# wangjiarui153/AIGV-Assessor

Measured on AMD Instinct MI355X. Metric: scored clips/sec (8-frame 448x448, InternVL2-8B stage-2 score eval), higher is better.
Workload: dtype bf16

## Files before the change

### aigv-assessor_amd/context.py

```python
from __future__ import annotations

import ctypes as C
from typing import Dict, Optional

import torch
import torch.nn.functional as F

from . import native
from .graphs import _PARKED_GRAPHS


def rope_tables(head_dim: int, theta: float, n_pos: int, max_pos: int = 32768, scaling: Optional[dict] = None,
                seq_len: Optional[int] = None):
    base = float(theta)
    if scaling is not None and scaling.get("type") == "dynamic" and seq_len is not None and seq_len > max_pos:
        f = float(scaling["factor"])
        base = base * ((f * seq_len / max_pos) - (f - 1)) ** (head_dim / (head_dim - 2))
    inv_freq = 1.0 / (base ** (torch.arange(0, head_dim, 2).float() / head_dim))
    t = torch.arange(n_pos).to(inv_freq.dtype)
    if scaling is not None and scaling.get("type") == "linear":
        t = t / float(scaling["factor"])
    freqs = torch.outer(t, inv_freq)
    return freqs.cos().to(torch.bfloat16).contiguous(), freqs.sin().to(torch.bfloat16).contiguous()

# ... 131 lines not shown
            if name.startswith("mlpscore.ln1"):
                continue
            if name == "vision_model.embeddings.position_embedding":
                put(name, resized_pos_table(p.data, v.image_size // v.patch_size, cfg.image_size // v.patch_size))
            else:
                put(name, p.data)
        if self.stage == 1:
            put("mlpscore.fc1.weight", torch.zeros(1, l.hidden_size, dtype=torch.bfloat16))
            put("mlpscore.fc1.bias", torch.zeros(1, dtype=torch.bfloat16))
        self._upload_rope()
        native.check(lib.aigv_finalize_weights(ctx), ctx)
        native.check(lib.aigv_set_precision(ctx, 1 if getattr(self, "_precision", "bf16") == "fp8" else 0), ctx)
        native.check(lib.aigv_set_gemm_mode(ctx, int(getattr(self, "_gemm_mode", -1))), ctx)
        native.check(lib.aigv_set_row_trimming(ctx, int(getattr(self, "_row_trim", True))), ctx)
        native.check(lib.aigv_set_attention_numerics(ctx, int(getattr(self, "_attn_numerics", 0))), ctx)
        self._dirty = False

    def __del__(self):
        try:
            _PARKED_GRAPHS.extend(v for v in getattr(self, "_graphs", {}).values() if isinstance(v, tuple))
        except Exception:
            pass
        try:
            if getattr(self, "_ctx", None) is not None:
                native.release("aigv_ctx_destroy", self._ctx)
        except Exception:
            pass

    def _ctx_set(self, entry: str, *args):
        lib, ctx = self._native()
        native.check(getattr(lib, entry)(ctx, *args), ctx)

    def set_precision(self, mode: str = "bf16"):
        self._drop_graphs()
        if mode not in ("bf16", "fp8"):
            raise ValueError("precision must be 'bf16' or 'fp8'")
        self._precision = mode
        if self._ctx is not None and not self._dirty:
            native.check(native.load().aigv_set_precision(self._ctx, 1 if mode == "fp8" else 0), self._ctx)

    def set_attention_numerics(self, mode: str = "fp32"):
        self._drop_graphs()
        if mode not in ("reference", "fp32"):
            raise ValueError("attention numerics must be 'reference' or 'fp32'")
        self._attn_numerics = 1 if mode == "reference" else 0
        self._ctx_set("aigv_set_attention_numerics", self._attn_numerics)

    def set_gemm_mode(self, mode: int = -1):
        self._drop_graphs()
        self._gemm_mode = int(mode)
        self._ctx_set("aigv_set_gemm_mode", int(mode))

    TUNE_KNOBS = {"gemm_mode": 0, "gemm256_order": 1, "gemm256_variant": 2, "attn_waves": 3, "skinny_p": 4, "body_tile": 5, "co_kmax": 6,
                  "tail_slices": 7, "attn_lead_key": 8, "decode_fused": 9, "decode_fp8": 10, "skinny_p8": 11, "fuse_tails": 12, "lone_body": 13}

    def tune(self, knob: str, value: int = -1):
        self._drop_graphs()
        self._ctx_set("aigv_ctx_tune", self.TUNE_KNOBS[knob], int(value))

    def set_row_trimming(self, on: bool = True):
        self._drop_graphs()
        self._row_trim = bool(on)
        self._ctx_set("aigv_set_row_trimming", int(on))
        self.drop_dead_tail = bool(on)

    def prof_enable(self, on: bool = True):
        self._drop_graphs()
        self._prof_on = bool(on)
        self._ctx_set("aigv_prof_enable", int(on))

    def prof_read(self) -> Dict[str, Dict[str, float]]:
        lib, ctx = self._native()
        out = {}
        for cls, name in enumerate(("gemm_llm", "attn_vit", "attn_llm", "skinny", "gemm_fp8", "gemm_vit")):
            n, ms, fl, by = C.c_int64(), C.c_double(), C.c_double(), C.c_double()
            native.check(lib.aigv_prof_read(ctx, cls, C.byref(n), C.byref(ms), C.byref(fl), C.byref(by)), ctx)
            out[name] = dict(launches=n.value, ms=ms.value, flops=fl.value, bytes=by.value)
        out["gemm"] = {k: out["gemm_llm"][k] + out["gemm_vit"][k] for k in out["gemm_llm"]}
        return out
```

### aigv-assessor_amd/csrc/ctx.h

```cpp
#pragma once
#include <hip/hip_runtime.h>

#include <algorithm>
#include <string>
#include <unordered_map>
#include <vector>

#include "../../include/aigv_amd.h"
#include "kernels.h"

namespace aigv {

struct DevBuf {
  void* p = nullptr;
  size_t bytes = 0;
};

struct VitLayer {
  const bf16_t *ls1, *ls2, *qkv_w, *qkv_b, *qn, *kn, *proj_w, *proj_b, *fc1_w, *fc1_b, *fc2_w, *fc2_b, *n1w, *n1b, *n2w, *n2b;
};
struct LlmLayer {
  const bf16_t *wqkv, *wo, *w13, *w2, *an, *fn;
};

struct LlmLayerFp8 {
  uint8_t *wqkv = nullptr, *wo = nullptr, *w13 = nullptr, *w2 = nullptr;
  float *s_wqkv = nullptr, *s_wo = nullptr, *s_w13 = nullptr, *s_w2 = nullptr;
};

struct ProfRec {
  int cls;
  hipEvent_t a, b;
  double flops, bytes;
};

struct RowPlan {
  struct Tiny { int row0, stride_rows, count; };
  std::vector<Tiny> tiny;
  int rows = 0, body_halves = 0, tail_halves = 0, tail_rows = 0;
  int32_t* d_tab = nullptr;
  int cap_halves = 0;
};

}

struct aigv_ctx {
  aigv_config cfg{};
  int device = 0;
  std::string err;
  std::unordered_map<std::string, aigv::DevBuf> w;
  std::vector<void*> allocs;
  std::vector<void*> ws_allocs;
  bool ws_phase = false;
  bool finalized = false;
  int np = 0, S = 0, Kp = 0, grid = 0, ntok = 0, proj_in = 0, qkv_out = 0, head_dim = 0, vit_head_dim = 0, g = 0;
  std::vector<aigv::VitLayer> vit;
  std::vector<aigv::LlmLayer> llm;
  const bf16_t *patch_w = nullptr, *patch_b = nullptr, *pos = nullptr, *cls_pos = nullptr;
  const bf16_t *tok_emb = nullptr, *final_norm = nullptr, *lm_head = nullptr, *rope_cos = nullptr, *rope_sin = nullptr;
  const bf16_t *p_ln_w[2] = {nullptr, nullptr}, *p_ln_b[2] = {nullptr, nullptr}, *p_w1[2] = {nullptr, nullptr},
               *p_b1[2] = {nullptr, nullptr}, *p_w2[2] = {nullptr, nullptr}, *p_b2[2] = {nullptr, nullptr};
  ScoreHeadArgs score{};
  bf16_t *v_col = nullptr, *v_x = nullptr, *v_t = nullptr, *v_qkv = nullptr, *v_ao = nullptr, *v_h = nullptr;
  int32_t* v_cu = nullptr;
  bf16_t *p_t = nullptr, *p_mid = nullptr;
  bf16_t *l_h = nullptr, *l_t = nullptr, *l_qkv = nullptr, *l_ao = nullptr, *l_ffn = nullptr, *l_rows = nullptr;
  int32_t *l_pos = nullptr, *l_seq = nullptr, *l_cu = nullptr, *l_rowidx = nullptr, *l_rowidx2 = nullptr, *l_kvlen = nullptr;
  unsigned long long* l_packed = nullptr;
  int32_t* l_neg1 = nullptr;
  bool fp8_llm = false;
  bool llm_lin_dirty = false;
  std::vector<aigv::LlmLayerFp8> llm8;
  uint8_t* q8 = nullptr;
  float* q8_scale = nullptr;
  aigv::RowPlan rp_vit, rp_llm;
  const aigv::RowPlan* cur_rp = nullptr;
  bool trim_last_layer = true;
  int attn_round_scores = AIGV_ATTENTION_NUMERICS_DEFAULT;
  int tune[AIGV_TUNE_COUNT];
  aigv_ctx() { std::fill(tune, tune + AIGV_TUNE_COUNT, -1); }
  size_t splitk_floats = 0;
  float* splitk_ws = nullptr;
  float* splitk_ws_vit = nullptr;
  bool on_vit_front = false;
  bf16_t* l_trim = nullptr;
  bf16_t* l_trim_h = nullptr;
  bf16_t* l_score_ws = nullptr;
  bf16_t* l_lp = nullptr;
  int lp_ldo = 0;
  bf16_t *kc = nullptr, *vc = nullptr;
  bf16_t *kc_alt = nullptr, *vc_alt = nullptr;
  int32_t* beam_ints = nullptr;
  uint64_t *kv_drop = nullptr, *kv_drop_alt = nullptr;
  int kv_drop_ld = 0;
  bool kv_masked = false;
  float* dec_ws = nullptr;
  float2* dec_lse = nullptr;
  bf16_t* dec_cand = nullptr;
  int32_t *dec_pos = nullptr, *dec_seq = nullptr, *dec_kvlen = nullptr, *dec_slot = nullptr;
  std::vector<int32_t> h_dec;
  std::vector<int32_t> h_pos, h_seq, h_rowidx, h_kvlen;
  int kv_seqs = 0;
  bool kv_valid = false;
  struct {
    bool armed = false;
    int n_rows = 0, n_seg = 0, ld_cached = 0;
    int32_t rows[AIGV_MAX_PROBE_ROWS];
    const int32_t *seg_new = nullptr, *seg_cached = nullptr;
    float* out = nullptr;
    float* tok = nullptr;
    int ld_tok = 0;
  } probe;
  struct {
    bool armed = false;
    const uint64_t* words = nullptr;
    const uint64_t* rows = nullptr;
    int ld = 0;
    int layer_begin = 0, layer_end = 0;
  } drop;
  struct {
    bool armed = false;
    int n_score = 0, n_token = 0;
    int32_t rows[2 * AIGV_MAX_LENS_ROWS];
    bf16_t *hidden = nullptr, *normed = nullptr;
    float* score = nullptr;
  } lens;
  int32_t* l_lensidx = nullptr;
  struct StreamRows {
// ... 72 lines not shown
    if (!on) return;
    hipEventRecord(r.b, s);
    c->recs.push_back(r);
  }
};

struct RowPlanScope {
  aigv_ctx* c;
  RowPlanScope(aigv_ctx* c_, const RowPlan* rp) : c(c_) { c->cur_rp = rp; }
  ~RowPlanScope() { c->cur_rp = nullptr; }
};

struct SplitkVitScope {
  aigv_ctx* c;
  explicit SplitkVitScope(aigv_ctx* c_) : c(c_) { c->on_vit_front = true; }
  ~SplitkVitScope() { c->on_vit_front = false; }
};

struct GemmClassScope {
  aigv_ctx* c;
  int keep;
  GemmClassScope(aigv_ctx* c_, int cls) : c(c_), keep(c_->gemm_cls) { c->gemm_cls = cls; }
  ~GemmClassScope() { c->gemm_cls = keep; }
};

struct Tune {
  int v[AIGV_TUNE_COUNT];
  constexpr int operator[](int knob) const { return v[knob]; }
};
extern Tune g_tune;
inline int tune_knob(const aigv_ctx* c, int knob) { return (c && c->tune[knob] >= 0) ? c->tune[knob] : g_tune.v[knob]; }
inline int resolved_gemm_mode(const aigv_ctx* c) { return tune_knob(c, AIGV_TUNE_GEMM_MODE); }
inline Tune tune_of(const aigv_ctx* c) {
  Tune t;
  for (int k = 0; k < AIGV_TUNE_COUNT; ++k) t.v[k] = tune_knob(c, k);
  return t;
}

GemmArgs gemm_args(const bf16_t* A, int lda, const bf16_t* W, int ldw, bf16_t* C, int ldc, int M, int N, int K);
int build_row_plan(aigv_ctx* c, RowPlan& rp, const int32_t* cu, int n_seq, hipStream_t s);
int launch_one(aigv_ctx* c, const GemmArgs& a, int epi, bool use256, hipStream_t s);
int run_gemm(aigv_ctx* c, const GemmArgs& a, int epi, hipStream_t s);
int run_gemm_rows(aigv_ctx* c, const GemmArgs& a, int epi, const RowPlan& rp, hipStream_t s);
int run_gemm_full(aigv_ctx* c, const GemmArgs& a, int epi, hipStream_t s);
int run_llm_gemm(aigv_ctx* c, const GemmArgs& a, int epi, hipStream_t s);
int run_gemm_fp8(aigv_ctx* c, const bf16_t* A, int lda, int K, const uint8_t* W8, const float* w_scale, bf16_t* C, int ldc, int T, int N,
                 int epi, const bf16_t* resid, int ldr, hipStream_t s);
const char* skinny_check(const bf16_t* x, int ldx, int R, const bf16_t* W, int ldw, int N, int K, const bf16_t* resid, int ldr,
                         const bf16_t* out, int ldo, int epi);
int run_skinny(aigv_ctx* c, const bf16_t* x, int ldx, int R, const bf16_t* W, int ldw, int N, int K, const bf16_t* bias,
               const bf16_t* resid, int ldr, bf16_t* out, int ldo, int epi, hipStream_t s, int p = 1);
constexpr size_t SPLITK_MAX_FLOATS = (size_t)64 << 20;
int splitk_scratch(aigv_ctx* c, size_t need_floats, float** out);

struct DisarmScope {
  aigv_ctx* c;
  explicit DisarmScope(aigv_ctx* c_) : c(c_) {}
  ~DisarmScope() { c->probe.armed = false; c->drop.armed = false; c->lens.armed = false; c->stream_cap.armed = false; c->stream_patch.armed = false;
                   c->head_cap.armed = false; c->head_patch.armed = false; c->head_scale.armed = false; }
};
int probe_plan(aigv_ctx* c, const char* op, const int32_t* cu, int B, const int32_t* off_host, ProbeArgs* out);
int probe_layer(aigv_ctx* c, const ProbeArgs& plan, int li, bool cache, hipStream_t s);
int stream_rows_check(aigv_ctx* c, const char* op, const int32_t* rows, int n, int T, int lo, int hi, int L);
extern double g_rate256;

}
```

### aigv-assessor_amd/csrc/dispatch.hip

```cpp
#include <atomic>
#include <mutex>

#include "ctx.h"

namespace aigv {

static GemmArgs tuned(const aigv_ctx* c, const GemmArgs& a) {
  GemmArgs b = a;
  b.order_sel = tune_knob(c, AIGV_TUNE_GEMM256_ORDER); b.variant_sel = tune_knob(c, AIGV_TUNE_GEMM256_VARIANT);
  return b;
}
double g_rate256 = 1.46;
constexpr double KT128 = 0.95, FIX128 = 6.0, LONE128 = 0.70, FIX256 = 9.0, LAUNCH_GAP = 2.0;

static std::atomic<unsigned> g_route{0};
static inline void took(unsigned bit) { g_route.fetch_or(bit, std::memory_order_relaxed); }

static double kt256() { return 2.0 * KT128 / g_rate256; }

static double t256(long row_tiles, int N, int nk) {
  if (row_tiles <= 0) return 0;
  const long tiles = row_tiles * (N / 256);
  return (double)((tiles + 255) / 256) * (nk * kt256() + FIX256);
}
static double t128_blocks(long blocks, double nk_each) {
  const double rt = nk_each * KT128 + FIX128;
  const long full = blocks / 512, part = blocks % 512;
  return full * rt + (part == 0 ? 0.0 : part <= 256 ? LONE128 * rt : rt);
}
static double t128(int rows, int N, int nk) { return rows <= 0 ? 0 : t128_blocks((long)((rows + 127) / 128) * (N / 128), nk); }
static double t_finalize(long rows, int N, int S) { return (double)rows * N * (4.0 * S + 4.0) / 3.0e6 + 3.0; }

constexpr int MAX_DEVICES = 64;
static float* g_op_splitk_ws[MAX_DEVICES] = {};
static std::mutex g_op_splitk_lock;

int splitk_scratch(aigv_ctx* c, size_t need_floats, float** out) {
  if (need_floats > SPLITK_MAX_FLOATS) return fail(c, AIGV_ERR_ARG, "split-K scratch: %zu floats exceed the planner's cap", need_floats);
  if (c) {
    if (need_floats > c->splitk_floats) return fail(c, AIGV_ERR_STATE, "split-K scratch: %zu floats exceed the context's %zu", need_floats, c->splitk_floats);
    *out = c->on_vit_front ? c->splitk_ws_vit : c->splitk_ws;
    return 0;
  }
  int dev = 0;
  HIPCHK(c, hipGetDevice(&dev));
  if (dev < 0 || dev >= MAX_DEVICES) return fail(c, AIGV_ERR_ARG, "device %d out of range", dev);
  std::lock_guard<std::mutex> g(g_op_splitk_lock);
  if (!g_op_splitk_ws[dev]) HIPCHK(c, hipMalloc((void**)&g_op_splitk_ws[dev], SPLITK_MAX_FLOATS * sizeof(float)));
  *out = g_op_splitk_ws[dev];
  return 0;
}
constexpr int SPLITS[] = {2, 3, 4, 6, 8};

static double best_split128(int rows, int N, int nk, int epi, int* S_out) {
  *S_out = 1;
  double best = t128(rows, N, nk);
  if (epi == EPI_PATCH) return best;
  const long tiles = (long)((rows + 127) / 128) * (N / 128);
  for (int S : SPLITS) {
    if (nk % S || nk / S < 4 || (size_t)S * rows * N > SPLITK_MAX_FLOATS) continue;
    const double t = t128_blocks(tiles * S, (double)nk / S) + t_finalize(rows, N, S) + LAUNCH_GAP;
    if (t < best) { best = t; *S_out = S; }
  }
  return best;
}
static double best_split256(long row_tiles, int N, int nk, int* S_out) {
  *S_out = 0;
  double best = 1e30;
  for (int S : SPLITS) {
    if (nk % S || nk / S < 4 || (size_t)S * row_tiles * 256 * N > SPLITK_MAX_FLOATS) continue;
    const long blocks = row_tiles * (N / 256) * S;
    const double t = (double)((blocks + 255) / 256) * ((double)nk / S * kt256() + FIX256) + t_finalize(row_tiles * 256, N, S) + LAUNCH_GAP;
    if (t < best) { best = t; *S_out = S; }
  }
  return best;
}

static int skinny_epi(int epi) {
  switch (epi) {
    case EPI_STORE: return SK_STORE;
    case EPI_GELU: return SK_GELU;
    case EPI_LS_RESID: return SK_LS_RESID;
    case EPI_RESID: return SK_RESID;
    case EPI_SWIGLU: return SK_SWIGLU;
  }
  return -1;
}
static double t_skinny(int rows, int N, int K) {
  if (rows <= 0) return 0;
  if (rows > 64 || K % 128) return 1e30;
// ... 137 lines not shown
      took(AIGV_ROUTE_SKINNY);
      hipError_t e = aigv_launch_skinny_gemm(bot.A, bot.lda, bot.M, bot.W, bot.ldw, bot.N, bot.K, bot.bias, bot.resid, bot.ldr,
                                            bot.C, bot.ldc, sk, s, bot.ls);
      if (e != hipSuccess) return fail(c, AIGV_ERR_HIP, "skinny remainder (M=%d N=%d K=%d): %s", bot.M, bot.N, bot.K, hipGetErrorString(e));
      return 0;
    }
    if (pl.last_slices > 1) return launch_splitk(c, bot, epi, pl.last_slices, false, s);
    return launch_one(c, bot, epi, false, s);
  }
  return 0;
}

constexpr int TINY_TAIL = 4;

int build_row_plan(aigv_ctx* c, RowPlan& rp, const int32_t* cu, int n_seq, hipStream_t s) {
  rp.tiny.clear();
  std::vector<int32_t> body, tail;
  bool uniform = true;
  for (int b = 1; b < n_seq; ++b) uniform = uniform && (cu[b + 1] - cu[b] == cu[1] - cu[0]);
  rp.tail_rows = 0;
  for (int b = 0; b < n_seq; ++b) {
    const int L = cu[b + 1] - cu[b], nb = L / 256, rem = L % 256, r0 = cu[b] + nb * 256;
    for (int j = 0; j < 2 * nb; ++j) { body.push_back(cu[b] + j * 128); body.push_back(128); }
    if (rem == 0) continue;
    if (rem <= TINY_TAIL) {
      if (!uniform) rp.tiny.push_back({r0, 1, rem});
      else if (b == 0)
        for (int j = 0; j < rem; ++j) rp.tiny.push_back({r0 + j, L, n_seq});
      continue;
    }
    tail.push_back(r0); tail.push_back(std::min(rem, 128));
    if (rem > 128) { tail.push_back(r0 + 128); tail.push_back(rem - 128); }
    rp.tail_rows += rem;
  }
  rp.body_halves = (int)body.size() / 2;
  rp.tail_halves = (int)tail.size() / 2;
  rp.rows = cu[n_seq];
  if (rp.body_halves + rp.tail_halves > rp.cap_halves)
    return fail(c, AIGV_ERR_STATE, "row plan: %d half tiles exceed the table's %d", rp.body_halves + rp.tail_halves, rp.cap_halves);
  body.insert(body.end(), tail.begin(), tail.end());
  if (!body.empty()) HIPCHK(c, aigv_launch_write_ints(body.data(), (int)body.size(), rp.d_tab, s));
  return 0;
}

static int tail_slices(int N, int K, int forced) {
  const int tn = N / 256, nk = K / 64;
  int best = 1;
  for (int S : {2, 4, 8})
    if (nk % S == 0 && nk / S >= 8 && 2 * tn * S <= 256) best = S;
  if (forced == 1 || (forced > 1 && nk % forced == 0 && nk / forced >= 4)) best = forced;
  return best;
}

static int launch_tab(aigv_ctx* c, const GemmArgs& a, int epi, const int32_t* tab, int halves, int rows, int S, hipStream_t s) {
  if (halves <= 0) return 0;
  GemmArgs b = tuned(c, a);
  b.row_tab = tab; b.tab_halves = halves;
  GEMM_PROF_ROWS(c, a, rows, s);
  if (S <= 1) {
    took(AIGV_ROUTE_TAB_256);
    HIPCHK(c, aigv_launch_gemm256(b, epi, s));
    return 0;
  }
  float* ws = nullptr;
  TRY(splitk_scratch(c, (size_t)S * ((halves + 1) / 2) * 256 * a.N, &ws));
  took(AIGV_ROUTE_TAB_SPLITK);
  HIPCHK(c, aigv_launch_gemm_splitk(b, epi, S, ws, s, true));
  return 0;
}

static int run_tiny_tails(aigv_ctx* c, const GemmArgs& a, int epi, const RowPlan& rp, hipStream_t s) {
  const int sk = skinny_epi(epi);
  for (const RowPlan::Tiny& t : rp.tiny) {
    if (sk < 0 || a.K % 128) return fail(c, AIGV_ERR_STATE, "no skinny form for epilogue %d / K=%d (tiny sequence tails)", epi, a.K);
    const size_t ldx = (size_t)t.stride_rows * a.lda, ldo = (size_t)t.stride_rows * a.ldc, ldr = (size_t)t.stride_rows * a.ldr;
    if (ldx > 0x7fffffffu || ldo > 0x7fffffffu || ldr > 0x7fffffffu) return fail(c, AIGV_ERR_STATE, "tiny-tail row stride overflows");
    for (int i0 = 0; i0 < t.count; i0 += 64) {
      const int R = std::min(64, t.count - i0);
      const size_t r0 = (size_t)t.row0 + (size_t)i0 * t.stride_rows;
      ProfScope ps(c, c ? c->gemm_cls : AIGV_PROF_GEMM, 2.0 * R * (double)a.N * a.K, 2.0 * (double)a.N * a.K, s);
      took(t.stride_rows == 1 ? AIGV_ROUTE_TINY : AIGV_ROUTE_TINY_STRIDED);
      hipError_t e = aigv_launch_skinny_gemm(a.A + r0 * a.lda, (int)ldx, R, a.W, a.ldw, a.N, a.K, a.bias, a.resid ? a.resid + r0 * a.ldr : nullptr,
                                            (int)ldr, a.C + r0 * a.ldc, (int)ldo, sk, s, a.ls, 0);
      if (e != hipSuccess) return fail(c, AIGV_ERR_HIP, "skinny tiny tails (R=%d N=%d K=%d): %s", R, a.N, a.K, hipGetErrorString(e));
    }
  }
  return 0;
}

int run_gemm_rows(aigv_ctx* c, const GemmArgs& a, int epi, const RowPlan& rp, hipStream_t s) {
  if (const char* m = aigv_gemm_check(a, epi)) return fail(c, AIGV_ERR_ARG, "%s (M=%d N=%d K=%d epi=%d)", m, a.M, a.N, a.K, epi);
  if (a.M != rp.rows) return fail(c, AIGV_ERR_STATE, "row plan covers %d rows, the GEMM has %d", rp.rows, a.M);
  const int mode = resolved_gemm_mode(c);
  if (mode == 3) return run_gemm(c, a, epi, s);
  if (mode == 4) return use_co(c, a, mode) ? launch_co(c, a, epi, s) : launch_one(c, a, epi, false, s);
  if (use_co(c, a, mode)) {
    if (rp.body_halves + rp.tail_halves > 0) {
      GemmArgs b = a;
      b.row_tab = rp.d_tab; b.tab_halves = rp.body_halves + rp.tail_halves;
      GEMM_PROF_ROWS(c, a, rp.body_halves * 128 + rp.tail_rows, s);
      took(AIGV_ROUTE_TAB_CO);
      HIPCHK(c, aigv_launch_gemmco(tuned(c, b), epi, s));
    }
    return run_tiny_tails(c, a, epi, rp, s);
  }
  if (mode == 1 || a.N < 256) return launch_one(c, a, epi, false, s);
  if (mode == 2 && a.N % 256 == 0) return launch_one(c, a, epi, true, s);
  if (a.N % 256) {
    if (epi == EPI_SWIGLU) return launch_one(c, a, epi, false, s);
    TRY(run_gemm_rows(c, col_slice(a, 0, a.N - 128), epi, rp, s));
    return launch_one(c, col_slice(a, a.N - 128, 128), epi, false, s);
  }
  const int S = tail_slices(a.N, a.K, tune_knob(c, AIGV_TUNE_TAIL_SLICES));
  const bool body128 = rp.body_halves > 0 && tune_knob(c, AIGV_TUNE_BODY_TILE) == 2;
  const bool tails_apart = rp.tail_halves > 0 && S > 1;
  const long body_tiles = (long)(rp.body_halves / 2) * (a.N / 256);
  const int lone_knob = tune_knob(c, AIGV_TUNE_LONE_BODY);
  const bool lone = !body128 && lone_knob != 1 && rp.body_halves > 0 && a.N % 128 == 0 &&
                    (lone_knob == 2 || (body_tiles <= 128 && (!tails_apart || a.K / 64 >= 128) && (lone_knob != 3 || tails_apart) && (lone_knob != 4 || !tails_apart)));
  if (lone) {
    GemmArgs b = tuned(c, a);
    b.row_tab = rp.d_tab; b.tab_halves = tails_apart ? rp.body_halves : rp.body_halves + rp.tail_halves;
    b.variant_sel = 7;
    GEMM_PROF_ROWS(c, a, rp.body_halves * 128 + (tails_apart ? 0 : rp.tail_rows), s);
    took(AIGV_ROUTE_TAB_LONE);
    HIPCHK(c, aigv_launch_gemmco(b, epi, s));
  } else if (body128) {
    {
      GemmArgs b = a;
      b.row_tab = rp.d_tab; b.tab_halves = rp.body_halves;
      GEMM_PROF_ROWS(c, a, rp.body_halves * 128, s);
      took(AIGV_ROUTE_TAB_128);
      HIPCHK(c, aigv_launch_gemm(b, epi, s));
    }
    if (rp.tail_halves > 0 && !tails_apart) TRY(launch_tab(c, a, epi, rp.d_tab + 2 * rp.body_halves, rp.tail_halves, rp.tail_rows, 1, s));
  } else if (!tails_apart) {
    TRY(launch_tab(c, a, epi, rp.d_tab, rp.body_halves + rp.tail_halves, rp.body_halves * 128 + rp.tail_rows, 1, s));
  } else {
    const int tn = a.N / 256;
    const long body_wg = (long)(rp.body_halves / 2) * tn, slice_wg = (long)((rp.tail_halves + 1) / 2) * tn * S;
    const size_t need = (size_t)S * ((rp.tail_halves + 1) / 2) * 256 * a.N;
    const int fuse_knob = tune_knob(c, AIGV_TUNE_FUSE_TAILS);
    const bool by_fill = body_wg % 256 != 0 && body_wg % 256 + slice_wg <= 320;
    if (!lone && rp.body_halves > 0 && (rp.body_halves & 1) == 0 && need <= (c ? c->splitk_floats : SPLITK_MAX_FLOATS) && fuse_knob != 1 && (by_fill || fuse_knob == 2)) {
      float* ws = nullptr;
      TRY(splitk_scratch(c, need, &ws));
      GemmArgs b = tuned(c, a);
      b.row_tab = rp.d_tab; b.tab_halves = rp.body_halves; b.fuse_tail_halves = rp.tail_halves; b.part = ws; b.k_slices = S;
      GEMM_PROF_ROWS(c, a, rp.body_halves * 128 + rp.tail_halves * 128, s);
      took(AIGV_ROUTE_TAB_FUSED);
      HIPCHK(c, aigv_launch_gemm256_fused(b, epi, s));
      GemmArgs f = a;
      f.row_tab = rp.d_tab + 2 * rp.body_halves; f.tab_halves = rp.tail_halves;
      HIPCHK(c, aigv_launch_gemm_finalize(f, epi, S, ws, s));
      return run_tiny_tails(c, a, epi, rp, s);
    }
    if (!lone) TRY(launch_tab(c, a, epi, rp.d_tab, rp.body_halves, rp.body_halves * 128, 1, s));
  }
  if (tails_apart) {
    const size_t per_pair = (size_t)S * 256 * a.N;
    const size_t cap = c ? c->splitk_floats : SPLITK_MAX_FLOATS;
    const int max_halves = (int)std::min<size_t>(cap / per_pair, 4096) * 2;
    if (max_halves < 2) return fail(c, AIGV_ERR_STATE, "split-K scratch too small for one tail tile (N=%d, %d slices)", a.N, S);
    for (int h0 = 0; h0 < rp.tail_halves; h0 += max_halves) {
      const int nh = std::min(max_halves, rp.tail_halves - h0);
      TRY(launch_tab(c, a, epi, rp.d_tab + 2 * (rp.body_halves + h0), nh, nh * 128, S, s));
    }
  }
  return run_tiny_tails(c, a, epi, rp, s);
}

int run_gemm_full(aigv_ctx* c, const GemmArgs& a, int epi, hipStream_t s) {
  if (const char* m = aigv_gemm_check(a, epi)) return fail(c, AIGV_ERR_ARG, "%s (M=%d N=%d K=%d epi=%d)", m, a.M, a.N, a.K, epi);
  const int mode = resolved_gemm_mode(c);
  if (use_co(c, a, mode)) return launch_co(c, a, epi, s);
  if (mode == 1 || a.N < 256 || (a.N % 256 && epi == EPI_SWIGLU)) return launch_one(c, a, epi, false, s);
  if (a.N % 256) {
    TRY(launch_one(c, col_slice(a, 0, a.N - 128), epi, true, s));
    return launch_one(c, col_slice(a, a.N - 128, 128), epi, false, s);
  }
  return launch_one(c, a, epi, true, s);
}

int run_llm_gemm(aigv_ctx* c, const GemmArgs& a, int epi, hipStream_t s) {
  return c->cur_rp ? run_gemm_rows(c, a, epi, *c->cur_rp, s) : run_gemm(c, a, epi, s);
}

GemmArgs gemm_args(const bf16_t* A, int lda, const bf16_t* W, int ldw, bf16_t* C, int ldc, int M, int N, int K) {
  GemmArgs a{};
  a.A = A; a.lda = lda; a.W = W; a.ldw = ldw; a.C = C; a.ldc = ldc; a.M = M; a.N = N; a.K = K;
  return a;
}

int run_gemm_fp8(aigv_ctx* c, const bf16_t* A, int lda, int K, const uint8_t* W8, const float* w_scale, bf16_t* C, int ldc, int T, int N,
                 int epi, const bf16_t* resid, int ldr, hipStream_t s) {
  hipError_t e = hipSuccess;
  if (A) {
    e = aigv_launch_quant_fp8_rows(A, lda, T, K, c->q8, K, c->q8_scale, s);
    if (e != hipSuccess) return fail(c, AIGV_ERR_HIP, "fp8 activation quantisation (T=%d K=%d): %s", T, K, hipGetErrorString(e));
  }
  GemmArgs a = tuned(c, GemmArgs{});
  a.A = (const bf16_t*)c->q8; a.lda = K; a.W = (const bf16_t*)W8; a.ldw = K; a.C = C; a.ldc = ldc; a.M = T; a.N = N; a.K = K;
  a.row_scale = c->q8_scale; a.col_scale = w_scale; a.resid = resid; a.ldr = ldr;
  ProfScope ps(c, AIGV_PROF_GEMM_FP8, 2.0 * T * (double)N * K, (double)T * K + (double)N * K + 2.0 * T * (epi == EPI_SWIGLU ? N / 2 : N), s);
  e = aigv_launch_gemm256_fp8(a, epi, s);
  if (e != hipSuccess) return fail(c, e == hipErrorInvalidValue ? AIGV_ERR_ARG : AIGV_ERR_HIP, "fp8 gemm (M=%d N=%d K=%d epi=%d): %s", T, N, K, epi, hipGetErrorString(e));
  return 0;
}


const char* skinny_check(const bf16_t* x, int ldx, int R, const bf16_t* W, int ldw, int N, int K, const bf16_t* resid, int ldr,
                         const bf16_t* out, int ldo, int epi) {
  if (R < 0 || N <= 0 || K <= 0) return "skinny gemm: empty problem";
  if (R > 64) return "skinny gemm: more than 64 rows";
  if (K % 128) return "skinny gemm: K must be a multiple of 128";
  if (!x || !W || !out) return "skinny gemm: null operand";
  if (ldx < K || ldw < K || (ldx % 8) || (ldw % 8)) return "skinny gemm: bad leading dimension (ldx and ldw: at least K, multiples of 8)";
  const int n_out = epi == SK_SWIGLU ? N / 2 : N;
  if (ldo < n_out) return "skinny gemm: ldo is below the output width (rows would overlap)";
  if (ldo % 4) return "skinny gemm: ldo must be a multiple of 4 (the kernel stores 8 bytes at out + row * ldo + n)";
  if ((epi == SK_RESID || epi == SK_LS_RESID) && !resid) return "skinny gemm: residual epilogue needs resid";
  if (resid && ldr < n_out) return "skinny gemm: ldr is below the width of the residual rows";
  if (resid && (ldr % 4)) return "skinny gemm: ldr must be a multiple of 4 (the kernel reads 8 bytes at resid + row * ldr + n)";
  return nullptr;
}

int run_skinny(aigv_ctx* c, const bf16_t* x, int ldx, int R, const bf16_t* W, int ldw, int N, int K, const bf16_t* bias,
               const bf16_t* resid, int ldr, bf16_t* out, int ldo, int epi, hipStream_t s, int p) {
  if (const char* m = skinny_check(x, ldx, R, W, ldw, N, K, resid, ldr, out, ldo, epi))
    return fail(c, AIGV_ERR_ARG, "%s (R=%d N=%d K=%d epi=%d)", m, R, N, K, epi);
  ProfScope ps(c, AIGV_PROF_SKINNY, 2.0 * R * (double)N * K, 2.0 * (double)N * K, s);
  hipError_t e = aigv_launch_skinny_gemm(x, ldx, R, W, ldw, N, K, bias, resid, ldr, out, ldo, epi, s, nullptr, p);
  if (e != hipSuccess) return fail(c, e == hipErrorInvalidValue ? AIGV_ERR_ARG : AIGV_ERR_HIP,
                                   "skinny gemm (R=%d N=%d K=%d epi=%d): %s", R, N, K, epi, hipGetErrorString(e));
  return 0;
}

}

using namespace aigv;

extern "C" int aigv_plan_gemm(int M, int N, int K, int epi, int* plan, double* est_us) {
  if (!plan || M <= 0 || N <= 0 || K <= 0 || N % 128 || K % 64 || epi < 0 || epi >= EPI_COUNT)
    return fail(nullptr, AIGV_ERR_ARG, "aigv_plan_gemm: bad problem M=%d N=%d K=%d epi=%d", M, N, K, epi);
  const int pmode = g_tune[AIGV_TUNE_GEMM_MODE] == 3 ? 0 : g_tune[AIGV_TUNE_GEMM_MODE];
  const int right = split_columns(M, N, K, epi, pmode);
  const GemmPlan pl = plan_gemm(M, N - right, K, epi, pmode);
  plan[6] = right;
  plan[0] = pl.top_tiles; plan[1] = pl.mid_tiles; plan[2] = pl.mid_slices; plan[3] = pl.last_rows; plan[4] = pl.last_kind;
  plan[5] = pl.last_slices;
  if (est_us) *est_us = pl.est_us + (right ? t128(M, right, K / 64) + LAUNCH_GAP : 0.0);
  return 0;
}

extern "C" int aigv_gemm_route(int clear) {
  return (int)(clear ? g_route.exchange(0, std::memory_order_relaxed) : g_route.load(std::memory_order_relaxed));
}
```

### aigv-assessor_amd/csrc/kernels.h

```cpp
#pragma once
#include <hip/hip_runtime.h>
#include <stdint.h>

typedef uint16_t bf16_t;

enum GemmEpilogue {
  EPI_STORE = 0,
  EPI_GELU = 1,
  EPI_LS_RESID = 2,
  EPI_RESID = 3,
  EPI_SWIGLU = 4,
  EPI_PATCH = 5,
  EPI_COUNT = 6,
  EPI_PARTIAL = 6
};

struct GemmArgs {
  const bf16_t* A; int lda;
  const bf16_t* W; int ldw;
  bf16_t* C; int ldc;
  const bf16_t* bias;
  const bf16_t* ls;
  const bf16_t* resid; int ldr;
  const bf16_t* pos;
  int M, N, K;
  int np;
  float* part;
  int k_slices;
  const float* row_scale;
  const float* col_scale;
  const int32_t* row_tab; int tab_halves;
  int fuse_tail_halves, fuse_body_wg;
  int order_sel, variant_sel;
  int order;
};

const char* aigv_gemm_check(const GemmArgs& a, int epi);
hipError_t aigv_launch_gemm(const GemmArgs& a, int epi, hipStream_t s);
hipError_t aigv_launch_gemm_splitk(const GemmArgs& a, int epi, int k_slices, float* ws, hipStream_t s, bool tile256 = false);
hipError_t aigv_launch_gemm256_partial(const GemmArgs& a, hipStream_t s);
hipError_t aigv_launch_gemm256_fp8(const GemmArgs& a, int epi, hipStream_t s);
hipError_t aigv_launch_gemm256_fp8_partial(const GemmArgs& a, hipStream_t s);
hipError_t aigv_launch_gemm_splitk_fp8(const GemmArgs& a, int epi, int k_slices, float* ws, hipStream_t s);
hipError_t aigv_launch_rmsnorm_quant_fp8(const bf16_t* x, int ldx, const bf16_t* w, uint8_t* q, int ldq, float* scale, int rows, int H, float eps,
                                         hipStream_t s);
hipError_t aigv_launch_quant_fp8_rows(const bf16_t* x, int ldx, int rows, int K, uint8_t* q, int ldq, float* scale, hipStream_t s);
bool aigv_gemm256_supported(const GemmArgs& a);
hipError_t aigv_launch_gemm256_fused(const GemmArgs& a, int epi, hipStream_t s);
hipError_t aigv_launch_gemm_finalize(const GemmArgs& a, int epi, int k_slices, const float* ws, hipStream_t s);
hipError_t aigv_launch_gemm256(const GemmArgs& a, int epi, hipStream_t s);
bool aigv_gemmco_supported(const GemmArgs& a);
hipError_t aigv_launch_gemmco(const GemmArgs& a, int epi, hipStream_t s);

struct AttnArgsUnmasked {
  const bf16_t* q; int ldq;
  const bf16_t* k; int ldk;
  const bf16_t* v; int ldv;
  bf16_t* o; int ldo;
  const int32_t* cu;
  int n_seq, max_len;
  int n_heads, n_kv_heads;
  int q_group_stride, kv_head_stride;
  int kv_len_offset;
  const int32_t* kv_off;
  size_t kv_seq_stride;
  int causal;
  float post_div;
  int round_scores;
  float q_prescale;
  const int32_t* rope_pos; const bf16_t* rope_cos; const bf16_t* rope_sin;
  int rope_pos_is_row;
  int q_tail;
  int uniform_len;
  int waves;
  int lead_key;
  int q_begin;
};
struct AttnArgsKeyDrop : AttnArgsUnmasked {
  const uint64_t* key_drop;
  int ld_drop;
};
struct AttnArgs : AttnArgsKeyDrop {
  const uint64_t* drop_rows;
};
const char* aigv_attn_check(const AttnArgs& a, int head_dim);
hipError_t aigv_launch_attention(const AttnArgs& a, int head_dim, hipStream_t s);
constexpr int AIGV_DECODE_KEYS_PER_CHUNK = 128;
constexpr int AIGV_DECODE_MAX_CHUNKS = 2048;
size_t aigv_attention_decode_ws_floats(int n_seq, int n_kv, int g, int cap);
hipError_t aigv_launch_attention_decode(const bf16_t* q, int ldq, int q_group_stride, const bf16_t* kc,
                                        const bf16_t* vc, const int32_t* kv_lens, int cap, bf16_t* o, int ldo,
                                        int n_seq, int n_kv, int g, int head_dim, float post_div, int max_kv_len,
                                        float* ws, hipStream_t s, const uint64_t* key_drop = nullptr, int ld_drop = 0);

#ifndef AIGV_MAX_ATTN_SEGMENTS
#define AIGV_MAX_ATTN_SEGMENTS 64
#endif
#ifndef AIGV_MAX_PROBE_ROWS
#define AIGV_MAX_PROBE_ROWS 64
#endif
#ifndef AIGV_MAX_KV_CAPACITY
#define AIGV_MAX_KV_CAPACITY 262144
#endif
struct ProbeRow { int32_t row, row0, seq, off; };
struct ProbeRowTab { ProbeRow r[AIGV_MAX_PROBE_ROWS]; };
struct ProbeArgs {
  const bf16_t* q; int ldq;
  const bf16_t* k; int ldk;
  int n_heads, n_kv_heads;
  int q_group_stride, kv_head_stride;
  size_t kv_seq_stride;
  float post_div;
  const bf16_t* rope_cos; const bf16_t* rope_sin;
  const int32_t* seg_new; const int32_t* seg_cached; int ld_cached;
  int n_seg;
  float* out; size_t out_row_stride;
  int n_rows;
  ProbeRowTab tab;
  float* tok; int ld_tok; size_t tok_row_stride;
};
const char* aigv_probe_check(const ProbeArgs& a, int head_dim, int total_rows, int max_pos);
hipError_t aigv_launch_attention_probe(const ProbeArgs& a, int head_dim, hipStream_t s);

hipError_t aigv_launch_layernorm(const bf16_t* x, int ldx, const bf16_t* w, const bf16_t* b, bf16_t* y, int ldy,
                                 int rows, int H, float eps, hipStream_t s);
hipError_t aigv_launch_rmsnorm(const bf16_t* x, int ldx, const bf16_t* w, bf16_t* y, int ldy, int rows, int H,
                               float eps, const int32_t* row_idx, hipStream_t s);
hipError_t aigv_launch_pixel_shuffle(const bf16_t* vit, int grid, int Hv, bf16_t* out, int frames, hipStream_t s);
hipError_t aigv_launch_im2col(const bf16_t* frames, int F, int C, int S, int P, int Kp, bf16_t* out, hipStream_t s);
hipError_t aigv_launch_gather_rows(const bf16_t* src, int ld, const int32_t* idx, int n, bf16_t* dst, int H, hipStream_t s);
hipError_t aigv_launch_lens_tap(const bf16_t* src, int ld, const int32_t* idx, int n, const bf16_t* w, bf16_t* raw, bf16_t* normed, int H, float eps,
                                hipStream_t s);
hipError_t aigv_launch_scatter_rows(const bf16_t* src, const int32_t* idx, int n, bf16_t* dst, int ld, int H, hipStream_t s);
hipError_t aigv_launch_stream_rows(bf16_t* stream, int ld, const int32_t* idx, int n, bf16_t* side, int n_depths, int depth, int H, bool to_stream,
                                   hipStream_t s);
#define AIGV_MAX_HEAD_BITS 64
enum { HEAD_CAPTURE = 0, HEAD_PATCH = 1, HEAD_SCALE = 2 };
struct HeadScales { float v[AIGV_MAX_HEAD_BITS]; };
hipError_t aigv_launch_head_rows(bf16_t* ao, int ld, const int32_t* idx, int n, bf16_t* side, int n_layers, int layer, int n_heads, int D, int mode,
                                 uint64_t heads, const float* scale, hipStream_t s);
hipError_t aigv_launch_cls_rows(const bf16_t* cls_pos, bf16_t* x, int F, int tokens_per_frame, int H, hipStream_t s);
hipError_t aigv_launch_rope(bf16_t* qkv, int ld, const int32_t* pos, const bf16_t* cos, const bf16_t* sin,
                            int tokens, int n_rot, int slots, int n_groups, int D, hipStream_t s, int first_rot = 0);
hipError_t aigv_launch_embed(const int64_t* ids, const int32_t* slot, const bf16_t* emb, const bf16_t* vis,
                             const bf16_t* motion, int n_vis, bf16_t* out, int tokens, int H, hipStream_t s);
enum { SK_STORE = 0, SK_RESID = 1, SK_SWIGLU = 2, SK_GELU = 3, SK_ARGMAX = 4, SK_RELU = 5, SK_LS_RESID = 6, SK_ROPE_KV = 7, SK_ARGMAX_LSE = 8, SK_ARGMAX_LSE_STORE = 9 };
hipError_t aigv_launch_skinny_gemm(const bf16_t* x, int ldx, int R, const bf16_t* W, int ldw, int N, int K,
                                   const bf16_t* bias, const bf16_t* resid, int ldr, bf16_t* out, int ldo, int epi,
                                   hipStream_t s, const bf16_t* ls = nullptr, int p = 1);
struct AigvRopeKv {
  const int32_t* pos; const int32_t* seq;
  const bf16_t* cos; const bf16_t* sin;
  bf16_t* kc; bf16_t* vc;
  int g, n_kv, cap;
};
bool aigv_skinny_fp8_supported(int K, bool with_norm);
hipError_t aigv_launch_skinny_fp8(const bf16_t* x, int ldx, int R, const uint8_t* W8, int ldw, const float* w_scale, int N, int K, const bf16_t* resid,
                                  int ldr, bf16_t* out, int ldo, int epi, const AigvRopeKv* rk, const bf16_t* norm_w, float eps, int p, hipStream_t s);
bool aigv_skinny_norm_fusable(int K);
hipError_t aigv_launch_skinny_swiglu_normed(const bf16_t* x, int ldx, int R, const bf16_t* W, int ldw, int N, int K, bf16_t* out, int ldo,
                                            const bf16_t* norm_w, float norm_eps, hipStream_t s, int p = 1);
hipError_t aigv_launch_skinny_rope_kv(const bf16_t* x, int ldx, int R, const bf16_t* W, int ldw, int N, int K, bf16_t* qkv, int ldo,
                                      const int32_t* pos, const int32_t* seq, const bf16_t* cos, const bf16_t* sin, bf16_t* kc, bf16_t* vc,
                                      int g, int n_kv, int cap, int head_dim, hipStream_t s, const bf16_t* norm_w = nullptr, float norm_eps = 0.f, int p = 1);
hipError_t aigv_launch_lm_head_argmax(const bf16_t* h, int R, int H, const bf16_t* W, int V,
                                      unsigned long long* packed, int64_t* out_idx, float* out_val, hipStream_t s);
#ifndef AIGV_MAX_CANDIDATES
#define AIGV_MAX_CANDIDATES 64
#endif
#ifndef AIGV_MAX_TOPK
#define AIGV_MAX_TOPK 16
#endif
size_t aigv_lm_head_lse_slots(int V);
size_t aigv_cand_logit_elems(int R);
hipError_t aigv_launch_lm_head_argmax_logprob(const bf16_t* h, int R, int H, const bf16_t* W, int V, unsigned long long* packed, float2* part,
                                              int64_t* out_idx, float* out_val, float* out_logprob, hipStream_t s, const int64_t* cand = nullptr,
                                              int C = 0, bf16_t* cand_logit = nullptr, float* out_cand = nullptr, int k = 0,
                                              bf16_t* row_logit = nullptr, int ldl = 0, int64_t* top_ids = nullptr, float* top_logprob = nullptr);
size_t aigv_topk_logit_ld(int V);
hipError_t aigv_launch_lm_head_lse_partials(const bf16_t* h, int R, int H, const bf16_t* W, int V, unsigned long long* packed, float2* part,
                                            hipStream_t s, bf16_t* logits = nullptr, int ldl = 0);
hipError_t aigv_launch_lm_head_logits(const bf16_t* h, int R, int H, const bf16_t* W, int V, bf16_t* out, int ldo, hipStream_t s,
                                      bool one_form = false, int ldh = 0);
hipError_t aigv_launch_label_logprob(const bf16_t* logits, int rows, int V, int ldo, const int64_t* labels, float* out, hipStream_t s);
hipError_t aigv_launch_cand_logprob(const bf16_t* logits, int rows, int V, int ldo, const int64_t* cand, int C, float* out, hipStream_t s);
hipError_t aigv_launch_topk_logprob(const bf16_t* logits, int rows, int V, int ldo, int k, int64_t* top_ids, float* top_logprob, hipStream_t s);
struct ScoreHeadArgs {
  const bf16_t* x; int ldx; int B;
  int n_layers; int dims[9];
  const bf16_t* w[8]; const bf16_t* b[8];
  float* score;
};
hipError_t aigv_launch_score_head(const ScoreHeadArgs& a, bf16_t* scratch, hipStream_t s);
hipError_t aigv_launch_score_head_groups(const ScoreHeadArgs& a, int G, size_t group_stride, bf16_t* scratch, hipStream_t s);
hipError_t aigv_launch_kv_store(const bf16_t* qkv, int ld, const int32_t* seq_of_tok, const int32_t* pos,
                                bf16_t* kc, bf16_t* vc, int tokens, int n_groups, int g, int D, int cap,
// ... 19 lines not shown
```

### aigv-assessor_amd/csrc/ops.hip

```cpp
#include "ctx.h"

using namespace aigv;

extern "C" {

int aigv_op_gemm(const void* A, int lda, const void* W_, int ldw, void* C, int ldc, const void* bias, const void* ls,
                 const void* resid, int ldr, const void* pos, int np, int M, int N, int K, int epi, void* stream) {
  GemmArgs a = gemm_args((const bf16_t*)A, lda, (const bf16_t*)W_, ldw, (bf16_t*)C, ldc, M, N, K);
  a.bias = (const bf16_t*)bias; a.ls = (const bf16_t*)ls; a.resid = (const bf16_t*)resid; a.ldr = ldr;
  a.pos = (const bf16_t*)pos; a.np = np;
  return run_gemm(nullptr, a, epi, (hipStream_t)stream);
}

int aigv_op_gemm_check(const void* A, int lda, const void* W_, int ldw, const void* C, int ldc, const void* bias, const void* ls,
                       const void* resid, int ldr, const void* pos, int np, int M, int N, int K, int epi) {
  GemmArgs a = gemm_args((const bf16_t*)A, lda, (const bf16_t*)W_, ldw, (bf16_t*)C, ldc, M, N, K);
  a.bias = (const bf16_t*)bias; a.ls = (const bf16_t*)ls; a.resid = (const bf16_t*)resid; a.ldr = ldr;
  a.pos = (const bf16_t*)pos; a.np = np;
  if (const char* m = aigv_gemm_check(a, epi)) return fail(nullptr, AIGV_ERR_ARG, "%s (M=%d N=%d K=%d epi=%d)", m, M, N, K, epi);
  return 0;
}

int aigv_op_skinny_gemm_check(const void* x, int ldx, int R, const void* W_, int ldw, int N, int K, const void* resid, int ldr,
                              const void* out, int ldo, int epi) {
  if (const char* m = skinny_check((const bf16_t*)x, ldx, R, (const bf16_t*)W_, ldw, N, K, (const bf16_t*)resid, ldr, (const bf16_t*)out, ldo, epi))
    return fail(nullptr, AIGV_ERR_ARG, "%s (R=%d N=%d K=%d epi=%d)", m, R, N, K, epi);
  return 0;
}

int aigv_op_gemm_rows(const void* A, int lda, const void* W_, int ldw, void* C, int ldc, const void* bias, const void* ls,
                      const void* resid, int ldr, const int32_t* cu_host, int n_seq, int N, int K, int epi, void* stream) {
  if (!cu_host || n_seq < 1 || cu_host[0] != 0) return fail(nullptr, AIGV_ERR_ARG, "aigv_op_gemm_rows: bad cu_seqlens");
  for (int b = 0; b < n_seq; ++b)
    if (cu_host[b + 1] <= cu_host[b]) return fail(nullptr, AIGV_ERR_ARG, "aigv_op_gemm_rows: empty sequence %d", b);
  if (epi == EPI_PATCH) return fail(nullptr, AIGV_ERR_ARG, "aigv_op_gemm_rows: no patch epilogue");
  const int M = cu_host[n_seq];
  GemmArgs a = gemm_args((const bf16_t*)A, lda, (const bf16_t*)W_, ldw, (bf16_t*)C, ldc, M, N, K);
  a.bias = (const bf16_t*)bias; a.ls = (const bf16_t*)ls; a.resid = (const bf16_t*)resid; a.ldr = ldr;
  RowPlan rp;
  rp.cap_halves = M / 128 + 2 * n_seq + 2;
  HIPCHK(nullptr, hipMalloc((void**)&rp.d_tab, (size_t)2 * rp.cap_halves * sizeof(int32_t)));
  int rc = build_row_plan(nullptr, rp, cu_host, n_seq, (hipStream_t)stream);
  if (!rc) rc = run_gemm_rows(nullptr, a, epi, rp, (hipStream_t)stream);
  hipStreamSynchronize((hipStream_t)stream);
  hipFree(rp.d_tab);
  return rc;
}

int aigv_op_gemm_splitk(const void* A, int lda, const void* W_, int ldw, void* C, int ldc, const void* bias, const void* ls,
                        const void* resid, int ldr, int M, int N, int K, int epi, int k_slices, void* ws_f32, void* stream) {
  GemmArgs a = gemm_args((const bf16_t*)A, lda, (const bf16_t*)W_, ldw, (bf16_t*)C, ldc, M, N, K);
  a.bias = (const bf16_t*)bias; a.ls = (const bf16_t*)ls; a.resid = (const bf16_t*)resid; a.ldr = ldr;
  if (const char* m = aigv_gemm_check(a, epi)) return fail(nullptr, AIGV_ERR_ARG, "%s", m);
  hipError_t e = aigv_launch_gemm_splitk(a, epi, k_slices, (float*)ws_f32, (hipStream_t)stream);
  if (e != hipSuccess) return fail(nullptr, e == hipErrorInvalidValue ? AIGV_ERR_ARG : AIGV_ERR_HIP, "split-K gemm: %s", hipGetErrorString(e));
  return 0;
}

int aigv_op_gemm_splitk256(const void* A, int lda, const void* W_, int ldw, void* C, int ldc, const void* bias, const void* ls,
                           const void* resid, int ldr, int M, int N, int K, int epi, int k_slices, void* ws_f32, void* stream) {
  GemmArgs a = gemm_args((const bf16_t*)A, lda, (const bf16_t*)W_, ldw, (bf16_t*)C, ldc, M, N, K);
  a.bias = (const bf16_t*)bias; a.ls = (const bf16_t*)ls; a.resid = (const bf16_t*)resid; a.ldr = ldr;
  if (const char* m = aigv_gemm_check(a, epi)) return fail(nullptr, AIGV_ERR_ARG, "%s", m);
  hipError_t e = aigv_launch_gemm_splitk(a, epi, k_slices, (float*)ws_f32, (hipStream_t)stream, true);
  if (e != hipSuccess) return fail(nullptr, e == hipErrorInvalidValue ? AIGV_ERR_ARG : AIGV_ERR_HIP, "split-K gemm (256 tile): %s", hipGetErrorString(e));
  return 0;
}

int aigv_op_quant_fp8_rows(const void* x_bf16, int ldx, int rows, int K, void* q_e4m3, int ldq, float* row_scale, void* stream) {
  hipError_t e = aigv_launch_quant_fp8_rows((const bf16_t*)x_bf16, ldx, rows, K, (uint8_t*)q_e4m3, ldq, row_scale, (hipStream_t)stream);
  if (e != hipSuccess) return fail(nullptr, e == hipErrorInvalidValue ? AIGV_ERR_ARG : AIGV_ERR_HIP, "fp8 row quantisation (rows=%d K=%d): %s", rows, K, hipGetErrorString(e));
  return 0;
}

int aigv_op_gemm_fp8(const void* A_e4m3, int lda, const void* W_e4m3, int ldw, void* C, int ldc, const float* row_scale,
                     const float* col_scale, const void* bias, const void* ls, const void* resid, int ldr, int M, int N, int K, int epi,
                     int k_slices, void* ws_f32, void* stream) {
  GemmArgs a{};
  a.A = (const bf16_t*)A_e4m3; a.lda = lda; a.W = (const bf16_t*)W_e4m3; a.ldw = ldw; a.C = (bf16_t*)C; a.ldc = ldc;
  a.M = M; a.N = N; a.K = K; a.bias = (const bf16_t*)bias; a.row_scale = row_scale; a.col_scale = col_scale;
  a.ls = (const bf16_t*)ls; a.resid = (const bf16_t*)resid; a.ldr = ldr;
  const int n_out = epi == EPI_SWIGLU ? N / 2 : N;
  if (ldc < n_out || (ldc % 8) || lda < K || ldw < K)
    return fail(nullptr, AIGV_ERR_ARG, "aigv_op_gemm_fp8: bad leading dimension (M=%d N=%d K=%d)", M, N, K);
  hipError_t e = k_slices > 1 ? aigv_launch_gemm_splitk_fp8(a, epi, k_slices, (float*)ws_f32, (hipStream_t)stream)
                              : aigv_launch_gemm256_fp8(a, epi, (hipStream_t)stream);
  if (e != hipSuccess)
    return fail(nullptr, e == hipErrorInvalidValue ? AIGV_ERR_ARG : AIGV_ERR_HIP,
                "fp8 gemm (M=%d N=%d K=%d epi=%d; needs N %% 256 == 0, K %% 128 == 0, 16-byte row strides, both scale vectors, epi in "
                "{store, gelu, ls_resid, resid, swiglu}): %s", M, N, K, epi, hipGetErrorString(e));
  return 0;
}

int aigv_op_skinny_gemm(const void* x, int ldx, int R, const void* W_, int ldw, int N, int K, const void* bias,
                        const void* resid, int ldr, void* out, int ldo, int epi, void* stream) {
  return run_skinny(nullptr, (const bf16_t*)x, ldx, R, (const bf16_t*)W_, ldw, N, K, (const bf16_t*)bias,
                    (const bf16_t*)resid, ldr, (bf16_t*)out, ldo, epi, (hipStream_t)stream, g_tune[AIGV_TUNE_SKINNY_P] ? g_tune[AIGV_TUNE_SKINNY_P] : 1);
}

// ... 600 lines not shown
```

### aigv-assessor_amd/csrc/passes.hip

```cpp
#include <cmath>

#include "ctx.h"

using namespace aigv;

namespace aigv {
int stream_rows_check(aigv_ctx* c, const char* op, const int32_t* rows, int n, int T, int lo, int hi, int L) {
  if (lo < 0 || lo > hi || hi > L) return fail(c, AIGV_ERR_ARG, "%s: depths [%d, %d) outside 0 <= lo <= hi <= %d", op, lo, hi, L);
  for (int i = 0; i < n; ++i) {
    if (rows[i] < 0 || rows[i] >= T) return fail(c, AIGV_ERR_ARG, "%s: row %d (packed row %d) outside [0, %d), the rows the pass runs", op, i, rows[i], T);
    if (i > 0 && rows[i] <= rows[i - 1])
      return fail(c, AIGV_ERR_ARG, "%s: rows %d and %d (packed rows %d, %d) are not strictly ascending", op, i - 1, i, rows[i - 1], rows[i]);
  }
  return 0;
}
}

extern "C" {

static int vit_norm(aigv_ctx* c, const bf16_t* x, const bf16_t* w, const bf16_t* b, bf16_t* y, int rows, hipStream_t s) {
  const aigv_config& k = c->cfg;
  if (k.vit_norm_rms) HIPCHK(c, aigv_launch_rmsnorm(x, k.vit_hidden, w, y, k.vit_hidden, rows, k.vit_hidden, k.vit_eps, nullptr, s));
  else HIPCHK(c, aigv_launch_layernorm(x, k.vit_hidden, w, b, y, k.vit_hidden, rows, k.vit_hidden, k.vit_eps, s));
  return 0;
// ... 116 lines not shown
  const aigv_config& k = c->cfg;
  const int H = k.llm_hidden, Md = k.motion_dim;
  if ((size_t)n_clips * Md > (size_t)k.vit_chunk * c->ntok * c->proj_in || n_clips > k.vit_chunk * c->ntok)
    return fail(c, AIGV_ERR_STATE, "motion batch does not fit the projector workspace");
  HIPCHK(c, aigv_launch_layernorm((const bf16_t*)motion_feature, Md, c->p_ln_w[1], c->p_ln_b[1], c->p_t, Md, n_clips, Md, 1e-5f, s));
  for (int r0 = 0; r0 < n_clips; r0 += 64) {
    const int R = std::min(64, n_clips - r0);
    TRY(run_skinny(c, c->p_t + (size_t)r0 * Md, Md, R, c->p_w1[1], Md, H, Md, c->p_b1[1], nullptr, 0,
                   c->p_mid + (size_t)r0 * H, H, SK_GELU, s, 0));
    TRY(run_skinny(c, c->p_mid + (size_t)r0 * H, H, R, c->p_w2[1], H, H, H, c->p_b2[1], nullptr, 0,
                   (bf16_t*)out + (size_t)r0 * H, H, SK_STORE, s, 0));
  }
  return 0;
}

static int upload_out_rows(aigv_ctx* c, const int32_t* score_rows, bool with_score, int B, const int32_t* logit_rows, int R,
                           int total_rows, hipStream_t s) {
  const aigv_config& k = c->cfg;
  if (R > k.max_out_rows) return fail(c, AIGV_ERR_ARG, "%d logit rows exceed max_out_rows %d", R, k.max_out_rows);
  c->h_rowidx.clear();
  for (int i = 0; i < (with_score ? B : 0); ++i) c->h_rowidx.push_back(score_rows[i]);
  for (int i = 0; i < R; ++i) c->h_rowidx.push_back(logit_rows[i]);
  for (int v : c->h_rowidx)
    if (v < 0 || v >= total_rows) return fail(c, AIGV_ERR_ARG, "output row index %d outside 0..%d", v, total_rows - 1);
  if (!c->h_rowidx.empty()) HIPCHK(c, aigv_launch_write_ints(c->h_rowidx.data(), (int)c->h_rowidx.size(), c->l_rowidx, s));
  return 0;
}

static int final_rows(aigv_ctx* c, float* score, int B, int R, int64_t* argmax, const bf16_t* hidden, bool compact, hipStream_t s) {
  const aigv_config& k = c->cfg;
  const int H = k.llm_hidden;
  const int nS = score ? B : 0;
  const int n = nS + R;
  if (n == 0) return 0;
  HIPCHK(c, aigv_launch_rmsnorm(hidden, H, c->final_norm, c->l_rows, H, n, H, k.rms_eps, compact ? nullptr : c->l_rowidx, s));
  for (int b0 = 0; b0 < nS; b0 += 64) {
    ScoreHeadArgs a = c->score;
    a.x = c->l_rows + (size_t)b0 * H; a.ldx = H; a.B = std::min(64, nS - b0); a.score = score + b0;
    HIPCHK(c, aigv_launch_score_head(a, c->l_score_ws, s));
  }
  for (int r0 = 0; r0 < R; r0 += 64) {
    const int rr = std::min(64, R - r0);
    ProfScope ps(c, AIGV_PROF_SKINNY, 2.0 * rr * (double)k.vocab * H, 2.0 * (double)k.vocab * H, s);
    HIPCHK(c, aigv_launch_lm_head_argmax(c->l_rows + (size_t)(nS + r0) * H, rr, H, c->lm_head, k.vocab, c->l_packed,
                                         argmax + r0, nullptr, s));
  }
  return 0;
}

static int llm_layer_qkv(aigv_ctx* c, int li, int T, hipStream_t s) {
  const aigv_config& k = c->cfg;
  const LlmLayer& L = c->llm[li];
  const int H = k.llm_hidden, D = c->head_dim, g = c->g, nkv = k.llm_kv_heads;
  if (c->fp8_llm) {
    HIPCHK(c, aigv_launch_rmsnorm_quant_fp8(c->l_h, H, L.an, c->q8, H, c->q8_scale, T, H, k.rms_eps, s));
    TRY(run_gemm_fp8(c, nullptr, H, H, c->llm8[li].wqkv, c->llm8[li].s_wqkv, c->l_qkv, c->qkv_out, T, c->qkv_out, EPI_STORE, nullptr, 0, s));
  } else {
    HIPCHK(c, aigv_launch_rmsnorm(c->l_h, H, L.an, c->l_t, H, T, H, k.rms_eps, nullptr, s));
    TRY(run_llm_gemm(c, gemm_args(c->l_t, H, L.wqkv, H, c->l_qkv, c->qkv_out, T, c->qkv_out, H), EPI_STORE, s));
  }
  HIPCHK(c, aigv_launch_rope(c->l_qkv, c->qkv_out, c->l_pos, c->rope_cos, c->rope_sin, T, 1, g + 2, nkv, D, s, g));
  return 0;
}

static int llm_layer_post(aigv_ctx* c, int li, int T, hipStream_t s) {
  const aigv_config& k = c->cfg;
  const LlmLayer& L = c->llm[li];
  const int H = k.llm_hidden, I = k.llm_inter;
  if (c->fp8_llm && li != k.llm_layers - 1) {
    const LlmLayerFp8& Q = c->llm8[li];
    TRY(run_gemm_fp8(c, c->l_ao, H, H, Q.wo, Q.s_wo, c->l_h, H, T, H, EPI_RESID, c->l_h, H, s));
    HIPCHK(c, aigv_launch_rmsnorm_quant_fp8(c->l_h, H, L.fn, c->q8, H, c->q8_scale, T, H, k.rms_eps, s));
    TRY(run_gemm_fp8(c, nullptr, H, H, Q.w13, Q.s_w13, c->l_ffn, I, T, 2 * I, EPI_SWIGLU, nullptr, 0, s));
    TRY(run_gemm_fp8(c, c->l_ffn, I, I, Q.w2, Q.s_w2, c->l_h, H, T, H, EPI_RESID, c->l_h, H, s));
    return 0;
  }
  {
    GemmArgs a = gemm_args(c->l_ao, H, L.wo, H, c->l_h, H, T, H, H);
    a.resid = c->l_h; a.ldr = H;
    TRY(run_llm_gemm(c, a, EPI_RESID, s));
  }
  HIPCHK(c, aigv_launch_rmsnorm(c->l_h, H, L.fn, c->l_t, H, T, H, k.rms_eps, nullptr, s));
  TRY(run_llm_gemm(c, gemm_args(c->l_t, H, L.w13, H, c->l_ffn, I, T, 2 * I, H), EPI_SWIGLU, s));
  GemmArgs a = gemm_args(c->l_ffn, I, L.w2, I, c->l_h, H, T, H, I);
  a.resid = c->l_h; a.ldr = H;
  TRY(run_llm_gemm(c, a, EPI_RESID, s));
  return 0;
}

static int upload_decode_state(aigv_ctx* c, int N, hipStream_t s) {
  c->h_dec.resize((size_t)4 * N);
  for (int i = 0; i < N; ++i) {
    const int len = c->h_kvlen[i];
    c->h_dec[i] = len; c->h_dec[N + i] = i; c->h_dec[2 * N + i] = len + 1; c->h_dec[3 * N + i] = -1;
  }
  HIPCHK(c, aigv_launch_write_ints(c->h_dec.data(), N, c->dec_pos, s));
  HIPCHK(c, aigv_launch_write_ints(c->h_dec.data() + N, N, c->dec_seq, s));
  HIPCHK(c, aigv_launch_write_ints(c->h_dec.data() + 2 * N, N, c->dec_kvlen, s));
  HIPCHK(c, aigv_launch_write_ints(c->h_dec.data() + 3 * N, N, c->dec_slot, s));
  c->kv_seqs = N;
  return 0;
}

static AttnArgs llm_attn_args(const aigv_ctx* c, int B) {
  const aigv_config& k = c->cfg;
  const int D = c->head_dim;
  AttnArgs a{};
  a.q = c->l_qkv; a.ldq = c->qkv_out;
  a.o = c->l_ao; a.ldo = k.llm_hidden;
  a.cu = c->l_cu; a.n_seq = B;
  a.n_heads = k.llm_heads; a.n_kv_heads = k.llm_kv_heads;
  a.q_group_stride = (c->g + 2) * D;
  a.causal = 1; a.post_div = sqrtf((float)D); a.q_prescale = 1.0f;
  a.round_scores = c->attn_round_scores; a.waves = tune_knob(c, AIGV_TUNE_ATTN_WAVES);
  a.rope_pos = c->l_pos; a.rope_cos = c->rope_cos; a.rope_sin = c->rope_sin;
  a.rope_pos_is_row = 1;
  return a;
}

int aigv_llm_prefill(aigv_ctx* c, const int64_t* ids, const int32_t* slot, const int32_t* cu, int B, const void* vis,
                     int n_vis, const void* motion, const int32_t* score_rows, float* score, const int32_t* logit_rows,
                     int R, int64_t* argmax, int keep_kv, void* stream) {
  if (!c || !ids || !slot || !cu) return fail(c, AIGV_ERR_ARG, "aigv_llm_prefill: null argument");
  const bool probing = c->probe.armed;
  const bool dropping = c->drop.armed;
  const bool lensing = c->lens.armed;
  const bool patching = c->stream_patch.armed;
  const bool capturing = c->stream_cap.armed;
  const bool h_scaling = c->head_scale.armed, h_patching = c->head_patch.armed, h_capturing = c->head_cap.armed;
  DisarmScope disarm(c);
  if (!c->finalized) return fail(c, AIGV_ERR_STATE, "aigv_llm_prefill: call aigv_finalize_weights first");
  if (dropping && probing) return fail(c, AIGV_ERR_ARG, "aigv_llm_prefill: a key-drop mask and the score-attention probe are both armed: the probe does not know the mask");
  const aigv_config& k = c->cfg;
  if (dropping && (c->drop.layer_begin < 0 || c->drop.layer_begin > c->drop.layer_end || c->drop.layer_end > k.llm_layers))
    return fail(c, AIGV_ERR_ARG, "aigv_llm_prefill: key-drop mask armed for layers [%d, %d), outside 0 <= begin <= end <= %d", c->drop.layer_begin, c->drop.layer_end, k.llm_layers);
  if (dropping && keep_kv && (c->drop.rows || c->drop.layer_begin != 0 || c->drop.layer_end != k.llm_layers))
    return fail(c, AIGV_ERR_ARG, "aigv_llm_prefill: keep_kv under a key-drop mask with row words or a partial layer window (aigv_key_drop_arm_ex): the mask kept "
                                 "beside the KV cache has neither");
  if (B <= 0 || B > k.max_seqs) return fail(c, AIGV_ERR_ARG, "n_clips %d outside 1..%d", B, k.max_seqs);
// ... 53 lines not shown
    }
  }
  HIPCHK(c, hipSetDevice(c->device));
  hipStream_t s = (hipStream_t)stream;
  const int H = k.llm_hidden, I = k.llm_inter, D = c->head_dim, g = c->g, nkv = k.llm_kv_heads;

  if (B + 1 > AIGV_SMALL_INTS / 2) return fail(c, AIGV_ERR_ARG, "at most %d clips per prefill call", AIGV_SMALL_INTS / 2 - 1);
  HIPCHK(c, aigv_launch_seqpos(cu, B, c->l_pos, c->l_seq, c->l_cu, T, s));
  TRY(build_row_plan(c, c->rp_llm, cu, B, s));
  RowPlanScope rps(c, &c->rp_llm);

  HIPCHK(c, aigv_launch_embed(ids, slot, c->tok_emb, (const bf16_t*)vis, (const bf16_t*)motion, n_vis, c->l_h, T, H, s));
  TRY(upload_out_rows(c, score_rows, score != nullptr, B, logit_rows, R, T, s));
  const int32_t* lens_idx = c->l_lensidx;
  auto lens_tap = [&](int depth, const bf16_t* src, const int32_t* idx) -> int {
    const size_t off = (size_t)depth * n_lens * H;
    HIPCHK(c, aigv_launch_lens_tap(src, H, idx, n_lens, c->final_norm, c->lens.hidden + off, c->lens.normed + off, H, k.rms_eps, s));
    return 0;
  };
  if (patching) HIPCHK(c, aigv_launch_write_ints(sp.rows.data(), (int)sp.rows.size(), c->l_streamidx, s));
  if (capturing) HIPCHK(c, aigv_launch_write_ints(sc.rows.data(), (int)sc.rows.size(), c->l_streamidx + k.max_tokens, s));
  if (h_scaling && !hs.all_rows) HIPCHK(c, aigv_launch_write_ints(hs.rows.data(), (int)hs.rows.size(), c->l_headidx, s));
  if (h_patching) HIPCHK(c, aigv_launch_write_ints(hp.rows.data(), (int)hp.rows.size(), c->l_headidx + k.max_tokens, s));
  if (h_capturing) HIPCHK(c, aigv_launch_write_ints(hc.rows.data(), (int)hc.rows.size(), c->l_headidx + 2 * (size_t)k.max_tokens, s));
  if (lensing) {
    HIPCHK(c, aigv_launch_write_ints(c->lens.rows, n_lens, c->l_lensidx, s));
    HIPCHK(c, aigv_launch_write_ints(lens_at, n_lens, c->l_lensidx + 2 * AIGV_MAX_LENS_ROWS, s));
  }
  const int n_out = (int)c->h_rowidx.size();
  int q_tail = 0;
  constexpr int TRIM_ROWS = 16;
  std::vector<int32_t> small_rows;
  {
    std::vector<int> per_clip(B, 0), clip_of(c->h_rowidx.size());
    for (size_t i = 0; i < c->h_rowidx.size(); ++i) {
      int b = 0;
      while (cu[b + 1] <= c->h_rowidx[i]) ++b;
      clip_of[i] = b;
      ++per_clip[b];
      q_tail = std::max(q_tail, cu[b + 1] - c->h_rowidx[i]);
    }
    for (size_t i = 0; i < c->h_rowidx.size(); ++i)
      if (per_clip[clip_of[i]] <= TRIM_ROWS) small_rows.push_back(c->h_rowidx[i]);
  }
  const bool trim_ok = c->trim_last_layer && n_out > 0 && H % 128 == 0 && I % 128 == 0;
  const bool trim = trim_ok && (int)small_rows.size() == n_out;
  const bool mixed = trim_ok && !trim && !small_rows.empty();
  if (mixed) HIPCHK(c, aigv_launch_write_ints(small_rows.data(), (int)small_rows.size(), c->l_rowidx2, s));
  ProbeArgs probe{};
  if (probing) TRY(probe_plan(c, "aigv_llm_prefill", cu, B, nullptr, &probe));
  double attn_flops = 0;
  for (int b = 0; b < B; ++b) { const double L = cu[b + 1] - cu[b]; attn_flops += 4.0 * (L * (L + 1) / 2) * D * k.llm_heads; }
  const size_t kv_layer = (size_t)k.max_seqs * nkv * k.kv_capacity * D;
  for (int li = 0; li < k.llm_layers; ++li) {
    const LlmLayer& L = c->llm[li];
    if (patching && li >= sp.lo && li < sp.hi)
      HIPCHK(c, aigv_launch_stream_rows(c->l_h, H, c->l_streamidx, (int)sp.rows.size(), sp.buf, sp.hi - sp.lo, li - sp.lo, H, true, s));
    if (capturing && li >= sc.lo && li < sc.hi)
      HIPCHK(c, aigv_launch_stream_rows(c->l_h, H, c->l_streamidx + k.max_tokens, (int)sc.rows.size(), sc.buf, sc.hi - sc.lo, li - sc.lo, H, false, s));
    if (lensing) TRY(lens_tap(li, c->l_h, lens_idx));
    TRY(llm_layer_qkv(c, li, T, s));
    if (keep_kv)
      HIPCHK(c, aigv_launch_kv_store(c->l_qkv, c->qkv_out, c->l_seq, c->l_pos, c->kc + li * kv_layer, c->vc + li * kv_layer, T,
                                     nkv, g, D, k.kv_capacity, s));
    if (probing) TRY(probe_layer(c, probe, li, false, s));
    if (n_out == 0 && c->trim_last_layer && li == k.llm_layers - 1) break;
    {
      AttnArgs a = llm_attn_args(c, B);
      a.k = c->l_qkv + (size_t)g * D; a.v = c->l_qkv + (size_t)(g + 1) * D;
      a.ldk = a.ldv = c->qkv_out; a.kv_head_stride = (g + 2) * D;
      a.max_len = max_len;
      const bool last_trim = trim && li == k.llm_layers - 1;
      a.q_tail = last_trim && !(h_capturing && li >= hc.lo && li < hc.hi && !hc.rows.empty()) ? q_tail : 0;
      if (dropping && li >= c->drop.layer_begin && li < c->drop.layer_end) { a.key_drop = c->drop.words; a.ld_drop = c->drop.ld; a.drop_rows = c->drop.rows; }
      if (const char* m = aigv_attn_check(a, D)) return fail(c, AIGV_ERR_ARG, "%s", m);
      ProfScope ps(c, AIGV_PROF_ATTN_LLM, last_trim ? 0.0 : attn_flops, 2.0 * T * ((double)c->qkv_out + H), s);
      HIPCHK(c, aigv_launch_attention(a, D, s));
    }
    if (h_scaling)
      HIPCHK(c, aigv_launch_head_rows(c->l_ao, H, hs.all_rows ? nullptr : c->l_headidx, hs.all_rows ? T : (int)hs.rows.size(), nullptr, 1, 0, k.llm_heads, D, HEAD_SCALE,
                                      ~(uint64_t)0, hs.scale.data() + (size_t)li * k.llm_heads, s));
    if (h_patching && li >= hp.lo && li < hp.hi)
      HIPCHK(c, aigv_launch_head_rows(c->l_ao, H, c->l_headidx + k.max_tokens, (int)hp.rows.size(), hp.buf, hp.hi - hp.lo, li - hp.lo, k.llm_heads, D, HEAD_PATCH,
                                      hp.bits[li - hp.lo], nullptr, s));
    if (h_capturing && li >= hc.lo && li < hc.hi)
      HIPCHK(c, aigv_launch_head_rows(c->l_ao, H, c->l_headidx + 2 * (size_t)k.max_tokens, (int)hc.rows.size(), hc.buf, hc.hi - hc.lo, li - hc.lo, k.llm_heads, D, HEAD_CAPTURE,
                                      ~(uint64_t)0, nullptr, s));
    if ((trim || mixed) && li == k.llm_layers - 1) {
      const int32_t* idx = trim ? c->l_rowidx : c->l_rowidx2;
      const int n_fin = trim ? n_out : (int)small_rows.size();
      bf16_t *t_ao = c->l_trim, *t_n = t_ao + (size_t)64 * H, *t_ffn = t_n + (size_t)64 * H, *t_h = c->l_trim_h;
      for (int r0 = 0; r0 < n_fin; r0 += 64) {
        const int nr = std::min(64, n_fin - r0);
        bf16_t* h = t_h + (size_t)r0 * H;
        HIPCHK(c, aigv_launch_gather_rows(c->l_ao, H, idx + r0, nr, t_ao, H, s));
        HIPCHK(c, aigv_launch_gather_rows(c->l_h, H, idx + r0, nr, h, H, s));
        TRY(run_skinny(c, t_ao, H, nr, L.wo, H, H, H, nullptr, h, H, h, H, SK_RESID, s, 0));
        HIPCHK(c, aigv_launch_rmsnorm(h, H, L.fn, t_n, H, nr, H, k.rms_eps, nullptr, s));
        TRY(run_skinny(c, t_n, H, nr, L.w13, H, 2 * I, H, nullptr, nullptr, 0, t_ffn, I, SK_SWIGLU, s, 0));
        TRY(run_skinny(c, t_ffn, I, nr, L.w2, I, H, I, nullptr, h, H, h, H, SK_RESID, s, 0));
      }
      if (trim) {
        if (lensing) TRY(lens_tap(k.llm_layers, t_h, lens_idx + 2 * AIGV_MAX_LENS_ROWS));
        TRY(final_rows(c, score, B, R, argmax, t_h, true, s));
        break;
      }
      TRY(llm_layer_post(c, li, T, s));
      HIPCHK(c, aigv_launch_scatter_rows(t_h, c->l_rowidx2, n_fin, c->l_h, H, H, s));
      if (lensing) TRY(lens_tap(k.llm_layers, c->l_h, lens_idx));
      break;
    }
    TRY(llm_layer_post(c, li, T, s));
    if (lensing && li == k.llm_layers - 1) TRY(lens_tap(k.llm_layers, c->l_h, lens_idx));
  }
  if (!trim) TRY(final_rows(c, score, B, R, argmax, c->l_h, false, s));
  if (lensing && c->lens.n_score > 0) {
    const int nS = c->lens.n_score, per = std::max(1, 64 / nS);
    for (int d0 = 0; d0 <= k.llm_layers; d0 += per) {
      ScoreHeadArgs a = c->score;
      a.x = c->lens.normed + (size_t)d0 * n_lens * H; a.ldx = H; a.B = nS; a.score = c->lens.score + (size_t)d0 * nS;
      HIPCHK(c, aigv_launch_score_head_groups(a, std::min(per, k.llm_layers + 1 - d0), (size_t)n_lens * H, c->l_score_ws, s));
    }
  }
  if (keep_kv) {
    c->h_kvlen.resize(B);
    for (int b = 0; b < B; ++b) c->h_kvlen[b] = cu[b + 1] - cu[b];
    TRY(upload_decode_state(c, B, s));
    if (dropping) HIPCHK(c, aigv_launch_kv_drop_rows(c->drop.words, c->drop.ld, nullptr, c->l_cu, 1, c->kv_drop, c->kv_drop_ld, B, s));
    c->kv_masked = dropping;
    c->kv_valid = true;
  } else {
    c->kv_valid = false;
    c->kv_masked = false;
  }
  return 0;
}

static int key_drop_arm(const char* op, aigv_ctx* c, const uint64_t* words_dev, const uint64_t* row_words_dev, int ld_words, int layer_begin, int layer_end) {
  if (!c) return fail(c, AIGV_ERR_ARG, "%s: null context", op);
  if (!words_dev || ((uintptr_t)words_dev & 7)) return fail(c, AIGV_ERR_ARG, "%s: words_dev is null or not 8-byte aligned", op);
  if ((uintptr_t)row_words_dev & 7) return fail(c, AIGV_ERR_ARG, "%s: row_words_dev is not 8-byte aligned", op);
  if (ld_words < 1) return fail(c, AIGV_ERR_ARG, "%s: ld_words = %d must be positive", op, ld_words);
  if (layer_begin < 0 || layer_begin > layer_end || layer_end > c->cfg.llm_layers)
    return fail(c, AIGV_ERR_ARG, "%s: layers [%d, %d) outside 0 <= begin <= end <= %d", op, layer_begin, layer_end, c->cfg.llm_layers);
  c->drop.words = words_dev; c->drop.rows = row_words_dev; c->drop.ld = ld_words;
  c->drop.layer_begin = layer_begin; c->drop.layer_end = layer_end;
  c->drop.armed = true;
  return 0;
}

int aigv_key_drop_arm(aigv_ctx* c, const uint64_t* words_dev, int ld_words) {
  if (!c) return fail(c, AIGV_ERR_ARG, "aigv_key_drop_arm: null context");
  return key_drop_arm("aigv_key_drop_arm", c, words_dev, nullptr, ld_words, 0, c->cfg.llm_layers);
}

int aigv_key_drop_arm_ex(aigv_ctx* c, const uint64_t* words_dev, const uint64_t* row_words_dev, int ld_words, int layer_begin, int layer_end) {
  return key_drop_arm("aigv_key_drop_arm_ex", c, words_dev, row_words_dev, ld_words, layer_begin, layer_end);
}

int aigv_depth_lens_arm(aigv_ctx* c, const int32_t* score_rows_host, int n_score, const int32_t* token_rows_host, int n_token, void* hidden_out_bf16,
                        void* normed_out_bf16, float* score_out) {
  const char* op = "aigv_depth_lens_arm";
  if (!c) return fail(c, AIGV_ERR_ARG, "%s: null context", op);
  if (n_score < 0 || n_score > AIGV_MAX_LENS_ROWS || n_token < 0 || n_token > AIGV_MAX_LENS_ROWS)
    return fail(c, AIGV_ERR_ARG, "%s: %d score rows and %d token rows: each list holds 0..%d rows", op, n_score, n_token, AIGV_MAX_LENS_ROWS);
  if (n_score + n_token == 0) return fail(c, AIGV_ERR_ARG, "%s: no row to read (n_score = n_token = 0)", op);
  if ((n_score > 0 && !score_rows_host) || (n_token > 0 && !token_rows_host)) return fail(c, AIGV_ERR_ARG, "%s: null row list", op);
// ... 62 lines not shown
  const size_t cells = (size_t)c->cfg.llm_layers * c->cfg.llm_heads;
  for (size_t i = 0; i < cells; ++i)
    if (scale_host[i] != scale_host[i])
      return fail(c, AIGV_ERR_ARG, "%s: scale[%d][%d] is NaN", op, (int)(i / c->cfg.llm_heads), (int)(i % c->cfg.llm_heads));
  TRY(head_rows_arm(op, c, &c->head_scale, rows_host, rows_host ? n : 0, 0, 0, nullptr, false));
  c->head_scale.scale.assign(scale_host, scale_host + cells);
  c->head_scale.lo = 0; c->head_scale.hi = c->cfg.llm_layers;
  c->head_scale.armed = true;
  return 0;
}

int aigv_llm_extend(aigv_ctx* c, const int64_t* ids, const int32_t* cu, int B, const int32_t* score_rows, float* score,
                    const int32_t* logit_rows, int R, int64_t* argmax, int commit, void* stream) {
  if (!c || !ids || !cu) return fail(c, AIGV_ERR_ARG, "aigv_llm_extend: null argument");
  const bool probing = c->probe.armed;
  const bool dropping = c->drop.armed;
  const bool lensing = c->lens.armed;
  const bool patching = c->stream_patch.armed, capturing = c->stream_cap.armed;
  const bool h_scaling = c->head_scale.armed, h_patching = c->head_patch.armed, h_capturing = c->head_cap.armed;
  DisarmScope disarm(c);
  if (h_scaling || h_patching || h_capturing)
    return fail(c, AIGV_ERR_ARG, "aigv_llm_extend: a head %s is armed (%s): the continuation pass takes none, only aigv_llm_prefill does", h_scaling ? "scale" : h_patching ? "patch" : "capture",
                h_scaling ? "aigv_head_scale_arm" : h_patching ? "aigv_head_patch_arm" : "aigv_head_capture_arm");
  if (patching || capturing)
    return fail(c, AIGV_ERR_ARG, "aigv_llm_extend: a stream %s is armed (%s): the continuation pass takes none, only aigv_llm_prefill does", patching ? "patch" : "capture",
                patching ? "aigv_stream_patch_arm" : "aigv_stream_capture_arm");
  if (lensing) return fail(c, AIGV_ERR_ARG, "aigv_llm_extend: the depth lens is armed (aigv_depth_lens_arm): the continuation pass takes no lens, only aigv_llm_prefill does");
  if (dropping) return fail(c, AIGV_ERR_ARG, "aigv_llm_extend: a key-drop mask is armed (aigv_key_drop_arm): the continuation pass takes no mask, only aigv_llm_prefill does");
  if (!c->kv_valid) return fail(c, AIGV_ERR_STATE, "aigv_llm_extend: no KV state (run aigv_llm_prefill with keep_kv)");
  if (probing && c->kv_masked) return fail(c, AIGV_ERR_ARG, "aigv_llm_extend: the score-attention probe is armed and the KV cache carries a key-drop mask: the probe does not know the mask");
  const aigv_config& k = c->cfg;
  if (B != c->kv_seqs) return fail(c, AIGV_ERR_ARG, "aigv_llm_extend: %d sequences, the cache holds %d", B, c->kv_seqs);
  if (B + 1 > AIGV_SMALL_INTS / 2) return fail(c, AIGV_ERR_ARG, "at most %d clips per call", AIGV_SMALL_INTS / 2 - 1);
  if (cu[0] != 0) return fail(c, AIGV_ERR_ARG, "cu_seqlens[0] must be 0");
  int max_new = 0, max_cached = 0;
  for (int b = 0; b < B; ++b) {
    const int n = cu[b + 1] - cu[b];
    max_cached = std::max(max_cached, (int)c->h_kvlen[b]);
    if (n <= 0) return fail(c, AIGV_ERR_ARG, "clip %d: no new tokens", b);
    if (c->h_kvlen[b] + n > k.kv_capacity || c->h_kvlen[b] + n > k.max_positions)
      return fail(c, AIGV_ERR_STATE, "clip %d: KV cache / RoPE table exhausted (%d cached + %d new, capacity %d)", b, c->h_kvlen[b], n, k.kv_capacity);
    max_new = std::max(max_new, n);
  }
  const int T = cu[B];
  if (T > k.max_tokens) return fail(c, AIGV_ERR_ARG, "%d new tokens exceed max_tokens %d", T, k.max_tokens);
  if ((score && !score_rows) || (R > 0 && (!logit_rows || !argmax))) return fail(c, AIGV_ERR_ARG, "output rows/buffers inconsistent");
  HIPCHK(c, hipSetDevice(c->device));
  hipStream_t s = (hipStream_t)stream;
  const int H = k.llm_hidden, D = c->head_dim, g = c->g, nkv = k.llm_kv_heads;
  HIPCHK(c, aigv_launch_seqpos(cu, B, c->l_pos, c->l_seq, c->l_cu, T, s, c->h_kvlen.data()));
  HIPCHK(c, aigv_launch_write_ints(c->h_kvlen.data(), B, c->l_kvlen, s));
  HIPCHK(c, aigv_launch_embed(ids, c->l_neg1, c->tok_emb, nullptr, nullptr, 0, c->l_h, T, H, s));
  TRY(upload_out_rows(c, score_rows, score != nullptr, B, logit_rows, R, T, s));
  ProbeArgs probe{};
  if (probing) TRY(probe_plan(c, "aigv_llm_extend", cu, B, c->h_kvlen.data(), &probe));
  double attn_flops = 0;
  for (int b = 0; b < B; ++b) { const double n = cu[b + 1] - cu[b]; attn_flops += 4.0 * n * (c->h_kvlen[b] + (n + 1) / 2) * D * k.llm_heads; }
  const size_t kv_layer = (size_t)k.max_seqs * nkv * k.kv_capacity * D;
  for (int li = 0; li < k.llm_layers; ++li) {
    TRY(llm_layer_qkv(c, li, T, s));
    HIPCHK(c, aigv_launch_kv_store(c->l_qkv, c->qkv_out, c->l_seq, c->l_pos, c->kc + li * kv_layer, c->vc + li * kv_layer, T, nkv, g, D,
                                   k.kv_capacity, s));
    if (probing) TRY(probe_layer(c, probe, li, true, s));
    {
      AttnArgs a = llm_attn_args(c, B);
      a.k = c->kc + li * kv_layer; a.v = c->vc + li * kv_layer;
      a.ldk = a.ldv = D; a.kv_head_stride = k.kv_capacity * D; a.kv_seq_stride = (size_t)nkv * k.kv_capacity * D;
      a.kv_off = c->l_kvlen;
      a.max_len = max_new;
      if (c->kv_masked) { a.key_drop = c->kv_drop; a.ld_drop = c->kv_drop_ld; a.kv_len_offset = max_cached; }
      if (const char* m = aigv_attn_check(a, D)) return fail(c, AIGV_ERR_ARG, "%s", m);
      ProfScope ps(c, AIGV_PROF_ATTN_LLM, attn_flops, 2.0 * T * ((double)c->qkv_out + H), s);
      HIPCHK(c, aigv_launch_attention(a, D, s));
    }
    TRY(llm_layer_post(c, li, T, s));
  }
  TRY(final_rows(c, score, B, R, argmax, c->l_h, false, s));
  if (commit) {
    for (int b = 0; b < B; ++b) {
      const int len = c->h_kvlen[b] + (cu[b + 1] - cu[b]);
      c->h_kvlen[b] = len;
      c->h_dec[b] = len; c->h_dec[2 * B + b] = len + 1;
    }
    HIPCHK(c, aigv_launch_write_ints(c->h_dec.data(), B, c->dec_pos, s));
    HIPCHK(c, aigv_launch_write_ints(c->h_dec.data() + 2 * B, B, c->dec_kvlen, s));
  }
  return 0;
}

int aigv_kv_fork(aigv_ctx* c, int copies, void* stream) {
  if (!c) return fail(c, AIGV_ERR_ARG, "aigv_kv_fork: null context");
  if (!c->kv_valid) return fail(c, AIGV_ERR_STATE, "aigv_kv_fork: no KV state (run aigv_llm_prefill with keep_kv)");
  const aigv_config& k = c->cfg;
  const int B = c->kv_seqs;
  if (copies < 1 || (long)B * copies > k.max_seqs) return fail(c, AIGV_ERR_ARG, "aigv_kv_fork: %d x %d sequences exceed max_seqs %d", B, copies, k.max_seqs);
  if (copies == 1) return 0;
  HIPCHK(c, hipSetDevice(c->device));
  hipStream_t s = (hipStream_t)stream;
  const size_t slot = (size_t)k.llm_kv_heads * k.kv_capacity * c->head_dim;
  const size_t kv_layer = (size_t)k.max_seqs * slot;
  for (int li = 0; li < k.llm_layers; ++li)
    for (int cpy = 1; cpy < copies; ++cpy) {
      HIPCHK(c, hipMemcpyAsync(c->kc + li * kv_layer + (size_t)cpy * B * slot, c->kc + li * kv_layer, (size_t)B * slot * sizeof(bf16_t), hipMemcpyDeviceToDevice, s));
      HIPCHK(c, hipMemcpyAsync(c->vc + li * kv_layer + (size_t)cpy * B * slot, c->vc + li * kv_layer, (size_t)B * slot * sizeof(bf16_t), hipMemcpyDeviceToDevice, s));
    }
  if (c->kv_masked)
// ... 304 lines not shown
```

### aigv-assessor_amd/csrc/rowops.hip

```cpp
#include <algorithm>
#include "common.h"
#include "kernels.h"

namespace {

constexpr int MAXC = 8;

__global__ __launch_bounds__(256) void layernorm_kernel(const bf16_t* __restrict__ x, int ldx,
                                                        const bf16_t* __restrict__ w, const bf16_t* __restrict__ b,
                                                        bf16_t* __restrict__ y, int ldy, int H, float eps) {
  __shared__ float red[4];
  const int row = blockIdx.x;
  const int nchunk = H >> 3;
  float v[MAXC][8];
  float sum = 0.f;
#pragma unroll
  for (int c = 0; c < MAXC; ++c) {
    const int ch = threadIdx.x + c * 256;
    if (ch < nchunk) {
      const u16x8 raw = *(const u16x8*)(x + (size_t)row * ldx + (ch << 3));
#pragma unroll
      for (int e = 0; e < 8; ++e) { v[c][e] = bf2f(raw[e]); sum += v[c][e]; }
    }
  }
  const float mean = block_sum_256(sum, red) / (float)H;
  float sq = 0.f;
#pragma unroll
  for (int c = 0; c < MAXC; ++c) {
    if (threadIdx.x + c * 256 < nchunk) {
#pragma unroll
      for (int e = 0; e < 8; ++e) { const float d = v[c][e] - mean; sq += d * d; }
    }
  }
  const float rstd = rsqrtf(block_sum_256(sq, red) / (float)H + eps);
#pragma unroll
  for (int c = 0; c < MAXC; ++c) {
    const int ch = threadIdx.x + c * 256;
    if (ch < nchunk) {
      const u16x8 ww = *(const u16x8*)(w + (ch << 3));
      const u16x8 bb = *(const u16x8*)(b + (ch << 3));
      u16x8 o;
#pragma unroll
      for (int e = 0; e < 8; ++e) o[e] = f2bf((v[c][e] - mean) * rstd * bf2f(ww[e]) + bf2f(bb[e]));
      *(u16x8*)(y + (size_t)row * ldy + (ch << 3)) = o;
    }
  }
}

template <int CH>
__global__ __launch_bounds__(256) void layernorm_wave_kernel(const bf16_t* __restrict__ x, int ldx,
                                                             const bf16_t* __restrict__ w, const bf16_t* __restrict__ b,
                                                             bf16_t* __restrict__ y, int ldy, int rows, float eps) {
  constexpr int H = 512 * CH;
  const int lane = threadIdx.x & 63;
// ... 18 lines not shown
  for (int c = 0; c < CH; ++c) {
    const int col = (lane + c * 64) << 3;
    const u16x8 ww = *(const u16x8*)(w + col);
    const u16x8 bb = *(const u16x8*)(b + col);
    u16x8 o;
#pragma unroll
    for (int e = 0; e < 8; ++e) o[e] = f2bf((v[c][e] - mean) * rstd * bf2f(ww[e]) + bf2f(bb[e]));
    *(u16x8*)(y + (size_t)row * ldy + col) = o;
  }
}

#define AIGV_RMSNORM_ROW(X, LDX, SROW, W, Y, LDY, ROW, H, EPS, KEEP_RAW)                          \
  __shared__ float red[4];                                                                        \
  const int nchunk = (H) >> 3;                                                                    \
  float v[MAXC][8];                                                                               \
  float sq = 0.f;                                                                                 \
  _Pragma("unroll") for (int c = 0; c < MAXC; ++c) {                                              \
    const int ch = threadIdx.x + c * 256;                                                         \
    if (ch < nchunk) {                                                                            \
      const u16x8 raw = *(const u16x8*)((X) + (size_t)(SROW) * (LDX) + (ch << 3));                \
      KEEP_RAW(ch, raw);                                                                          \
      _Pragma("unroll") for (int e = 0; e < 8; ++e) { v[c][e] = bf2f(raw[e]); sq += v[c][e] * v[c][e]; } \
    }                                                                                             \
  }                                                                                               \
  const float rstd = rsqrtf(block_sum_256(sq, red) / (float)(H) + (EPS));                         \
  _Pragma("unroll") for (int c = 0; c < MAXC; ++c) {                                              \
    const int ch = threadIdx.x + c * 256;                                                         \
    if (ch < nchunk) {                                                                            \
      const u16x8 ww = *(const u16x8*)((W) + (ch << 3));                                          \
      u16x8 o;                                                                                    \
      _Pragma("unroll") for (int e = 0; e < 8; ++e) o[e] = f2bf(bf2f(ww[e]) * rbf(v[c][e] * rstd)); \
      *(u16x8*)((Y) + (size_t)(ROW) * (LDY) + (ch << 3)) = o;                                     \
    }                                                                                             \
  }
#define AIGV_RMSNORM_NO_RAW(ch, raw) (void)0

__global__ __launch_bounds__(256) void rmsnorm_kernel(const bf16_t* __restrict__ x, int ldx,
                                                      const bf16_t* __restrict__ w, bf16_t* __restrict__ y, int ldy,
                                                      int H, float eps, const int32_t* __restrict__ row_idx) {
  const int row = blockIdx.x;
  const int srow = row_idx ? row_idx[row] : row;
  AIGV_RMSNORM_ROW(x, ldx, srow, w, y, ldy, row, H, eps, AIGV_RMSNORM_NO_RAW)
}

__global__ __launch_bounds__(256) void lens_tap_kernel(const bf16_t* __restrict__ src, int ld, const int32_t* __restrict__ idx,
                                                       const bf16_t* __restrict__ w, bf16_t* __restrict__ raw_out, bf16_t* __restrict__ normed,
                                                       int H, float eps) {
  const int row = blockIdx.x;
  const int srow = idx[row];
#define AIGV_LENS_KEEP_RAW(ch, raw) *(u16x8*)(raw_out + (size_t)row * H + (ch << 3)) = raw
  AIGV_RMSNORM_ROW(src, ld, srow, w, normed, H, row, H, eps, AIGV_LENS_KEEP_RAW)
#undef AIGV_LENS_KEEP_RAW
}
#undef AIGV_RMSNORM_ROW
#undef AIGV_RMSNORM_NO_RAW

__global__ __launch_bounds__(256) void rmsnorm_quant_fp8_kernel(const bf16_t* __restrict__ x, int ldx, const bf16_t* __restrict__ w,
                                                                uint8_t* __restrict__ q, int ldq, float* __restrict__ scale, int H, float eps) {
  __shared__ float red[4];
  __shared__ float redm[4];
  const int row = blockIdx.x;
  const int nchunk = H >> 3;
  float v[MAXC][8];
  float sq = 0.f;
#pragma unroll
  for (int c = 0; c < MAXC; ++c) {
    const int ch = threadIdx.x + c * 256;
    if (ch < nchunk) {
      const u16x8 raw = *(const u16x8*)(x + (size_t)row * ldx + (ch << 3));
#pragma unroll
      for (int e = 0; e < 8; ++e) { v[c][e] = bf2f(raw[e]); sq += v[c][e] * v[c][e]; }
    }
  }
  const float rstd = rsqrtf(block_sum_256(sq, red) / (float)H + eps);
  float amax = 0.f;
#pragma unroll
  for (int c = 0; c < MAXC; ++c) {
    const int ch = threadIdx.x + c * 256;
    if (ch < nchunk) {
      const u16x8 ww = *(const u16x8*)(w + (ch << 3));
#pragma unroll
      for (int e = 0; e < 8; ++e) {
        v[c][e] = rbf(bf2f(ww[e]) * rbf(v[c][e] * rstd));
        amax = fmaxf(amax, fabsf(v[c][e]));
      }
    }
  }
  amax = wave_max(amax);
  if ((threadIdx.x & 63) == 0) redm[threadIdx.x >> 6] = amax;
  __syncthreads();
  amax = fmaxf(fmaxf(redm[0], redm[1]), fmaxf(redm[2], redm[3]));
  const float inv = amax > 0.f ? __fdiv_rn(448.0f, amax) : 1.0f;
  if (threadIdx.x == 0) scale[row] = amax > 0.f ? __fdiv_rn(amax, 448.0f) : 1.0f;
#pragma unroll
  for (int c = 0; c < MAXC; ++c) {
    const int ch = threadIdx.x + c * 256;
    if (ch < nchunk) {
      int lo = 0, hi = 0;
      lo = __builtin_amdgcn_cvt_pk_fp8_f32(v[c][0] * inv, v[c][1] * inv, lo, false);
      lo = __builtin_amdgcn_cvt_pk_fp8_f32(v[c][2] * inv, v[c][3] * inv, lo, true);
      hi = __builtin_amdgcn_cvt_pk_fp8_f32(v[c][4] * inv, v[c][5] * inv, hi, false);
      hi = __builtin_amdgcn_cvt_pk_fp8_f32(v[c][6] * inv, v[c][7] * inv, hi, true);
      typedef __attribute__((ext_vector_type(2))) int i32x2;
      *(i32x2*)(q + (size_t)row * ldq + (ch << 3)) = i32x2{lo, hi};
    }
  }
// ... 60 lines not shown
    else *(u16x8*)(brow + (c << 3)) = *(const u16x8*)(srow + (c << 3));
  }
}

template <int MODE>
__global__ __launch_bounds__(256) void head_rows_kernel(bf16_t* __restrict__ ao, int ld, const int32_t* __restrict__ idx, bf16_t* __restrict__ side,
                                                        int n_layers, int layer, int H, int d_shift, uint64_t heads, const HeadScales scale) {
  const int i = blockIdx.x;
  bf16_t* arow = ao + (size_t)(idx ? idx[i] : i) * ld;
  bf16_t* brow = MODE == HEAD_SCALE ? nullptr : side + ((size_t)i * n_layers + layer) * H;
  for (int c = threadIdx.x; c < (H >> 3); c += 256) {
    const int h = (c << 3) >> d_shift;
    if (!((heads >> h) & 1)) continue;
    if (MODE == HEAD_CAPTURE) *(u16x8*)(brow + (c << 3)) = *(const u16x8*)(arow + (c << 3));
    else if (MODE == HEAD_PATCH) *(u16x8*)(arow + (c << 3)) = *(const u16x8*)(brow + (c << 3));
    else {
      const float f = scale.v[h];
      u16x8 x = *(const u16x8*)(arow + (c << 3));
#pragma unroll
      for (int e = 0; e < 8; ++e) x[e] = f2bf(bf2f(x[e]) * f);
      *(u16x8*)(arow + (c << 3)) = x;
    }
  }
}

__global__ __launch_bounds__(256) void rope_kernel(bf16_t* __restrict__ qkv, int ld, const int32_t* __restrict__ pos,
                                                   const bf16_t* __restrict__ cs, const bf16_t* __restrict__ sn,
                                                   int tokens, int n_rot, int slots, int n_groups, int D, int first_rot) {
  const int half = D >> 1, cph = half >> 3;
  const int per_tok = n_groups * n_rot * cph;
  const size_t total = (size_t)tokens * per_tok;
  for (size_t i = (size_t)blockIdx.x * blockDim.x + threadIdx.x; i < total; i += (size_t)gridDim.x * blockDim.x) {
    const int t = (int)(i / per_tok);
    int r = (int)(i - (size_t)t * per_tok);
    const int c = r % cph; r /= cph;
    const int s = r % n_rot, gidx = r / n_rot;
    bf16_t* base = qkv + (size_t)t * ld + (size_t)(gidx * slots + first_rot + s) * D + (c << 3);
    const size_t tb = (size_t)pos[t] * half + (c << 3);
    const u16x8 lo = *(const u16x8*)base, hi = *(const u16x8*)(base + half);
    const u16x8 co = *(const u16x8*)(cs + tb), si = *(const u16x8*)(sn + tb);
    u16x8 olo, ohi;
#pragma unroll
    for (int e = 0; e < 8; ++e) {
      bf16_t a, b;
      rope_pair(lo[e], hi[e], co[e], si[e], a, b);
      olo[e] = a;
      ohi[e] = b;
    }
    *(u16x8*)base = olo;
    *(u16x8*)(base + half) = ohi;
  }
}

__global__ __launch_bounds__(256) void embed_kernel(const int64_t* __restrict__ ids, const int32_t* __restrict__ slot,
                                                    const bf16_t* __restrict__ emb, const bf16_t* __restrict__ vis,
                                                    const bf16_t* __restrict__ motion, int n_vis,
                                                    bf16_t* __restrict__ out, int H) {
  const int t = blockIdx.x;
  const int s = slot[t];
  const bf16_t* src = s < 0 ? emb + (size_t)ids[t] * H : (s < n_vis ? vis + (size_t)s * H : motion + (size_t)(s - n_vis) * H);
  for (int c = threadIdx.x; c < (H >> 3); c += 256)
    *(u16x8*)(out + (size_t)t * H + (c << 3)) = *(const u16x8*)(src + (c << 3));
}

__global__ __launch_bounds__(256) void kv_store_kernel(const bf16_t* __restrict__ qkv, int ld,
                                                       const int32_t* __restrict__ seq_of_tok,
                                                       const int32_t* __restrict__ pos, bf16_t* __restrict__ kc,
                                                       bf16_t* __restrict__ vc, int n_groups, int g, int D, int cap) {
  const int t = blockIdx.x;
  const int sq = seq_of_tok[t], p = pos[t];
  const int cpd = D >> 3;
  for (int i = threadIdx.x; i < n_groups * 2 * cpd; i += 256) {
    const int c = i % cpd, r = i / cpd, which = r & 1, h = r >> 1;
    const bf16_t* src = qkv + (size_t)t * ld + (size_t)(h * (g + 2) + g + which) * D + (c << 3);
    bf16_t* dst = (which ? vc : kc) + (((size_t)sq * n_groups + h) * cap + p) * D + (c << 3);
    *(u16x8*)dst = *(const u16x8*)src;
  }
}

__global__ __launch_bounds__(256) void quant_fp8_rows_kernel(const bf16_t* __restrict__ x, int ldx, int K, uint8_t* __restrict__ q,
                                                             int ldq, float* __restrict__ scale) {
  __shared__ float red[4];
  const int row = blockIdx.x, lane = threadIdx.x & 63, wave = threadIdx.x >> 6;
  const bf16_t* xr = x + (size_t)row * ldx;
  float amax = 0.f;
  for (int c = threadIdx.x; c < (K >> 3); c += 256) {
    const u16x8 v = *(const u16x8*)(xr + (c << 3));
#pragma unroll
    for (int e = 0; e < 8; ++e) amax = fmaxf(amax, fabsf(bf2f(v[e])));
  }
  amax = wave_max(amax);
  if (lane == 0) red[wave] = amax;
  __syncthreads();
  amax = fmaxf(fmaxf(red[0], red[1]), fmaxf(red[2], red[3]));
  const float inv = amax > 0.f ? __fdiv_rn(448.0f, amax) : 1.0f;
  if (threadIdx.x == 0) scale[row] = amax > 0.f ? __fdiv_rn(amax, 448.0f) : 1.0f;
  uint8_t* qr = q + (size_t)row * ldq;
  for (int c = threadIdx.x; c < (K >> 3); c += 256) {
    const u16x8 v = *(const u16x8*)(xr + (c << 3));
    int lo = 0, hi = 0;
    lo = __builtin_amdgcn_cvt_pk_fp8_f32(bf2f(v[0]) * inv, bf2f(v[1]) * inv, lo, false);
    lo = __builtin_amdgcn_cvt_pk_fp8_f32(bf2f(v[2]) * inv, bf2f(v[3]) * inv, lo, true);
    hi = __builtin_amdgcn_cvt_pk_fp8_f32(bf2f(v[4]) * inv, bf2f(v[5]) * inv, hi, false);
    hi = __builtin_amdgcn_cvt_pk_fp8_f32(bf2f(v[6]) * inv, bf2f(v[7]) * inv, hi, true);
    typedef __attribute__((ext_vector_type(2))) int i32x2;
    *(i32x2*)(qr + (c << 3)) = i32x2{lo, hi};
// ... 93 lines not shown
  uint64_t word = 0;
  if (w < ld_src && live > 0) {
    word = src[(size_t)(parent ? parent[i] : i) * ld_src + w];
    if (live < 64) word &= (1ull << live) - 1;
  }
  dst[idx] = word;
}
}

hipError_t aigv_launch_kv_drop_rows(const uint64_t* src, int ld_src, const int32_t* parent, const int32_t* lens, int lens_are_cu, uint64_t* dst, int ld_dst,
                                    int n, hipStream_t s) {
  if (!src || !lens || !dst || src == dst || ld_src < 1 || ld_dst < 1 || n < 1) return hipErrorInvalidValue;
  hipLaunchKernelGGL(kv_drop_rows_kernel, dim3((n * ld_dst + 255) / 256), dim3(256), 0, s, src, ld_src, parent, lens, lens_are_cu, dst, ld_dst, n);
  return hipGetLastError();
}

hipError_t aigv_launch_write_ints(const int32_t* host, int n, int32_t* dst, hipStream_t s) {
  if (n <= 0) return hipSuccess;
  for (int off = 0; off < n; off += AIGV_SMALL_INTS) {
    SmallInts a{};
    const int m = n - off < AIGV_SMALL_INTS ? n - off : AIGV_SMALL_INTS;
    for (int i = 0; i < m; ++i) a.v[i] = host[off + i];
    hipLaunchKernelGGL(write_ints_kernel, dim3(1), dim3(AIGV_SMALL_INTS), 0, s, a, m, dst + off);
  }
  return hipGetLastError();
}

hipError_t aigv_launch_decode_eos(int64_t* tok, int32_t* state, int n, const int64_t* eos_host, int n_eos, int64_t pad, hipStream_t s) {
  if (n <= 0 || n > 64 || n_eos < 0 || n_eos > 8 || !tok || !state || (n_eos > 0 && !eos_host)) return hipErrorInvalidValue;
  EosIds e{};
  e.n = n_eos;
  for (int k = 0; k < n_eos; ++k) e.v[k] = (long long)eos_host[k];
  hipLaunchKernelGGL(decode_eos_kernel, dim3(1), dim3(64), 0, s, (long long*)tok, state, n, e, (long long)pad);
  return hipGetLastError();
}

hipError_t aigv_launch_advance(int32_t* a, int32_t* b, int n, hipStream_t s) {
  if (n <= 0 || n > 1024) return hipErrorInvalidValue;
  hipLaunchKernelGGL(advance_kernel, dim3(1), dim3(1024), 0, s, a, b, n);
  return hipGetLastError();
}

hipError_t aigv_launch_layernorm(const bf16_t* x, int ldx, const bf16_t* w, const bf16_t* b, bf16_t* y, int ldy,
                                 int rows, int H, float eps, hipStream_t s) {
  if (rows <= 0) return hipSuccess;
  if (H % 8 || H > MAXC * 256 * 8) return hipErrorInvalidValue;
  if (H == 1024) hipLaunchKernelGGL(layernorm_wave_kernel<2>, dim3((rows + 3) / 4), dim3(256), 0, s, x, ldx, w, b, y, ldy, rows, eps);
  else if (H == 2048) hipLaunchKernelGGL(layernorm_wave_kernel<4>, dim3((rows + 3) / 4), dim3(256), 0, s, x, ldx, w, b, y, ldy, rows, eps);
  else hipLaunchKernelGGL(layernorm_kernel, dim3(rows), dim3(256), 0, s, x, ldx, w, b, y, ldy, H, eps);
  return hipGetLastError();
}

hipError_t aigv_launch_rmsnorm(const bf16_t* x, int ldx, const bf16_t* w, bf16_t* y, int ldy, int rows, int H,
                               float eps, const int32_t* row_idx, hipStream_t s) {
  if (rows <= 0) return hipSuccess;
  if (H % 8 || H > MAXC * 256 * 8) return hipErrorInvalidValue;
  hipLaunchKernelGGL(rmsnorm_kernel, dim3(rows), dim3(256), 0, s, x, ldx, w, y, ldy, H, eps, row_idx);
  return hipGetLastError();
}

hipError_t aigv_launch_lens_tap(const bf16_t* src, int ld, const int32_t* idx, int n, const bf16_t* w, bf16_t* raw, bf16_t* normed, int H, float eps,
                                hipStream_t s) {
  if (n <= 0) return hipSuccess;
  if (H % 8 || H > MAXC * 256 * 8 || ld % 8 || ld < H || !src || !idx || !w || !raw || !normed) return hipErrorInvalidValue;
  hipLaunchKernelGGL(lens_tap_kernel, dim3(n), dim3(256), 0, s, src, ld, idx, w, raw, normed, H, eps);
  return hipGetLastError();
}

hipError_t aigv_launch_rmsnorm_quant_fp8(const bf16_t* x, int ldx, const bf16_t* w, uint8_t* q, int ldq, float* scale, int rows, int H, float eps,
                                         hipStream_t s) {
  if (rows <= 0) return hipSuccess;
  if (H % 8 || H > MAXC * 256 * 8 || ldq % 8 || !q || !scale) return hipErrorInvalidValue;
  hipLaunchKernelGGL(rmsnorm_quant_fp8_kernel, dim3(rows), dim3(256), 0, s, x, ldx, w, q, ldq, scale, H, eps);
  return hipGetLastError();
}

hipError_t aigv_launch_pixel_shuffle(const bf16_t* vit, int grid, int Hv, bf16_t* out, int frames, hipStream_t s) {
  if (frames <= 0) return hipSuccess;
  if (Hv % 8 || grid % 2) return hipErrorInvalidValue;
  const int rows = frames * (grid / 2) * (grid / 2);
  hipLaunchKernelGGL(pixel_shuffle_kernel, dim3(2048), dim3(256), 0, s, vit, grid, Hv, out, rows);
  return hipGetLastError();
}

hipError_t aigv_launch_im2col(const bf16_t* frames, int F, int C, int S, int P, int Kp, bf16_t* out, hipStream_t s) {
  if (F <= 0) return hipSuccess;
  if (S % P || Kp < C * P * P) return hipErrorInvalidValue;
  const int g = S / P;
  hipLaunchKernelGGL(im2col_kernel, dim3(F * g * g), dim3(256), 0, s, frames, C, S, P, Kp, out);
  return hipGetLastError();
}

hipError_t aigv_launch_cls_rows(const bf16_t* cls_pos, bf16_t* x, int F, int tokens_per_frame, int H, hipStream_t s) {
  if (F <= 0) return hipSuccess;
  hipLaunchKernelGGL(cls_rows_kernel, dim3(F), dim3(128), 0, s, cls_pos, x, tokens_per_frame, H);
  return hipGetLastError();
}

hipError_t aigv_launch_gather_rows(const bf16_t* src, int ld, const int32_t* idx, int n, bf16_t* dst, int H, hipStream_t s) {
  if (n <= 0) return hipSuccess;
  if (H % 8 || ld % 8) return hipErrorInvalidValue;
  hipLaunchKernelGGL(gather_rows_kernel, dim3(n), dim3(256), 0, s, src, ld, idx, dst, H);
  return hipGetLastError();
}

hipError_t aigv_launch_scatter_rows(const bf16_t* src, const int32_t* idx, int n, bf16_t* dst, int ld, int H, hipStream_t s) {
  if (n <= 0) return hipSuccess;
  if (H % 8 || ld % 8) return hipErrorInvalidValue;
  hipLaunchKernelGGL(scatter_rows_kernel, dim3(n), dim3(256), 0, s, src, idx, dst, ld, H);
  return hipGetLastError();
}

hipError_t aigv_launch_stream_rows(bf16_t* stream, int ld, const int32_t* idx, int n, bf16_t* side, int n_depths, int depth, int H, bool to_stream,
                                   hipStream_t s) {
  if (n <= 0) return hipSuccess;
  if (H < 8 || H % 8 || H > MAXC * 256 * 8 || ld % 8 || ld < H || n_depths < 1 || depth < 0 || depth >= n_depths || !stream || !idx || !side ||
      ((uintptr_t)stream & 15) || ((uintptr_t)side & 15))
    return hipErrorInvalidValue;
  if (to_stream) hipLaunchKernelGGL(stream_rows_kernel<true>, dim3(n), dim3(256), 0, s, stream, ld, idx, side, n_depths, depth, H);
  else hipLaunchKernelGGL(stream_rows_kernel<false>, dim3(n), dim3(256), 0, s, stream, ld, idx, side, n_depths, depth, H);
  return hipGetLastError();
}

hipError_t aigv_launch_head_rows(bf16_t* ao, int ld, const int32_t* idx, int n, bf16_t* side, int n_layers, int layer, int n_heads, int D, int mode,
                                 uint64_t heads, const float* scale, hipStream_t s) {
  if (n <= 0) return hipSuccess;
  const int H = n_heads * D;
  if (n_heads < 1 || n_heads > AIGV_MAX_HEAD_BITS || (D != 64 && D != 128) || ld % 8 || ld < H || !ao || ((uintptr_t)ao & 15)) return hipErrorInvalidValue;
  if (mode == HEAD_SCALE ? !scale : (!idx || !side || ((uintptr_t)side & 15) || n_layers < 1 || layer < 0 || layer >= n_layers)) return hipErrorInvalidValue;
  if (n_heads < 64) heads &= ((uint64_t)1 << n_heads) - 1;
  const int d_shift = D == 64 ? 6 : 7;
  HeadScales sc{};
  if (mode == HEAD_SCALE)
    for (int h = 0; h < n_heads; ++h) {
      sc.v[h] = scale[h];
      if (scale[h] == 1.0f) heads &= ~((uint64_t)1 << h);
    }
  if (!heads) return hipSuccess;
  if (mode == HEAD_CAPTURE) hipLaunchKernelGGL(head_rows_kernel<HEAD_CAPTURE>, dim3(n), dim3(256), 0, s, ao, ld, idx, side, n_layers, layer, H, d_shift, heads, sc);
  else if (mode == HEAD_PATCH) hipLaunchKernelGGL(head_rows_kernel<HEAD_PATCH>, dim3(n), dim3(256), 0, s, ao, ld, idx, side, n_layers, layer, H, d_shift, heads, sc);
  else if (mode == HEAD_SCALE) hipLaunchKernelGGL(head_rows_kernel<HEAD_SCALE>, dim3(n), dim3(256), 0, s, ao, ld, idx, side, 1, 0, H, d_shift, heads, sc);
  else return hipErrorInvalidValue;
  return hipGetLastError();
}

hipError_t aigv_launch_rope(bf16_t* qkv, int ld, const int32_t* pos, const bf16_t* cos, const bf16_t* sin,
                            int tokens, int n_rot, int slots, int n_groups, int D, hipStream_t s, int first_rot) {
  if (tokens <= 0 || n_rot <= 0) return hipSuccess;
  if (D % 16 || first_rot < 0 || first_rot + n_rot > slots) return hipErrorInvalidValue;
  const size_t total = (size_t)tokens * n_groups * n_rot * (D / 16);
  const int blocks = (int)((total + 255) / 256 < 4096 ? (total + 255) / 256 : 4096);
  hipLaunchKernelGGL(rope_kernel, dim3(blocks), dim3(256), 0, s, qkv, ld, pos, cos, sin, tokens, n_rot, slots,
                     n_groups, D, first_rot);
  return hipGetLastError();
}

hipError_t aigv_launch_quant_fp8_rows(const bf16_t* x, int ldx, int rows, int K, uint8_t* q, int ldq, float* scale, hipStream_t s) {
  if (rows <= 0) return hipSuccess;
  if (K <= 0 || K % 8 || ldx % 8 || ldq % 8 || !x || !q || !scale) return hipErrorInvalidValue;
  hipLaunchKernelGGL(quant_fp8_rows_kernel, dim3(rows), dim3(256), 0, s, x, ldx, K, q, ldq, scale);
  return hipGetLastError();
}

hipError_t aigv_launch_embed(const int64_t* ids, const int32_t* slot, const bf16_t* emb, const bf16_t* vis,
                             const bf16_t* motion, int n_vis, bf16_t* out, int tokens, int H, hipStream_t s) {
  if (tokens <= 0) return hipSuccess;
  if (H % 8) return hipErrorInvalidValue;
  hipLaunchKernelGGL(embed_kernel, dim3(tokens), dim3(256), 0, s, ids, slot, emb, vis, motion, n_vis, out, H);
  return hipGetLastError();
}

hipError_t aigv_launch_kv_store(const bf16_t* qkv, int ld, const int32_t* seq_of_tok, const int32_t* pos,
                                bf16_t* kc, bf16_t* vc, int tokens, int n_groups, int g, int D, int cap,
                                hipStream_t s) {
  if (tokens <= 0) return hipSuccess;
  hipLaunchKernelGGL(kv_store_kernel, dim3(tokens), dim3(256), 0, s, qkv, ld, seq_of_tok, pos, kc, vc, n_groups, g, D,
                     cap);
  return hipGetLastError();
}
```

### aigv-assessor_amd/csrc/tune.hip

```cpp
#include "ctx.h"

using namespace aigv;

namespace {

constexpr bool in_waves(int v) { return v == 0 || v == 4 || v == 8; }
constexpr bool in_forms(int v) { return v == 0 || v == 1 || v == 2 || v == 4; }
constexpr bool in_forms_packed(int v) { return in_forms(v) || (v >= 1000 && v < 1000 + 4096); }
constexpr bool in_kmax(int v) { return v >= 0 && v <= 65536 && v % 64 == 0; }

struct Knob {
  int def;
  int hi;
  bool (*in_set)(int);
  bool process_default;
};
constexpr Knob KNOBS[AIGV_TUNE_COUNT] = {
    {0, 4, nullptr, false},
    {0, 15, nullptr, false},
    {0, 7, nullptr, false},
    {0, 0, in_waves, false},
    {0, 0, in_forms_packed, false},
    {0, 2, nullptr, false},
    {0, 0, in_kmax, true},
    {0, 16, nullptr, true},
    {0, 1, nullptr, true},
    {1, 1, nullptr, false},
    {1, 1, nullptr, false},
    {0, 0, in_forms, false},
    {0, 2, nullptr, true},
    {1, 4, nullptr, true},
};
static_assert(AIGV_TUNE_GEMM_MODE == 0 && AIGV_TUNE_CO_KMAX == 6 && AIGV_TUNE_LONE_BODY == 13 && AIGV_TUNE_COUNT == 14, "KNOBS follows the enum's order");

constexpr Tune library_defaults() {
  Tune t{};
  for (int k = 0; k < AIGV_TUNE_COUNT; ++k) t.v[k] = KNOBS[k].def;
  return t;
}

bool known(int knob) { return knob >= 0 && knob < AIGV_TUNE_COUNT; }
bool valid(int knob, int value) { return KNOBS[knob].in_set ? KNOBS[knob].in_set(value) : value >= 0 && value <= KNOBS[knob].hi; }

}

Tune aigv::g_tune = library_defaults();

extern "C" {

int aigv_set_row_trimming(aigv_ctx* c, int on) {
  if (!c) return fail(c, AIGV_ERR_ARG, "aigv_set_row_trimming: null context");
  c->trim_last_layer = on != 0;
  return 0;
}

int aigv_get_attention_numerics(const aigv_ctx* c) { return c ? c->attn_round_scores : AIGV_ATTENTION_NUMERICS_DEFAULT; }

int aigv_set_attention_numerics(aigv_ctx* c, int mode) {
  if (!c) return fail(c, AIGV_ERR_ARG, "aigv_set_attention_numerics: null context");
  if (mode != 0 && mode != 1) return fail(c, AIGV_ERR_ARG, "aigv_set_attention_numerics: 0 (fp32 scores) or 1 (the reference's bf16 score matrix)");
  c->attn_round_scores = mode;
  return 0;
}

int aigv_set_gemm_mode(aigv_ctx* c, int mode) {
  if (!c) return fail(c, AIGV_ERR_ARG, "aigv_set_gemm_mode: null context");
  if (mode != -1 && !valid(AIGV_TUNE_GEMM_MODE, mode)) return fail(c, AIGV_ERR_ARG, "aigv_set_gemm_mode: mode must be -1 (process default), 0 (row plans), 1 (128 tile), 2 (256 tile), 3 (batch-level dispatch) or 4 (co-resident 256x128 tile)");
  c->tune[AIGV_TUNE_GEMM_MODE] = mode;
  return 0;
}

int aigv_ctx_tune(aigv_ctx* c, int knob, int value) {
  if (!c) return fail(c, AIGV_ERR_ARG, "aigv_ctx_tune: null context");
  if (knob == AIGV_TUNE_GEMM_MODE) return aigv_set_gemm_mode(c, value);
  if (!known(knob)) return fail(c, AIGV_ERR_ARG, "aigv_ctx_tune: unknown knob %d", knob);
  if (value != -1 && !valid(knob, value)) return fail(c, AIGV_ERR_ARG, "aigv_ctx_tune: value %d out of range for knob %d", value, knob);
  c->tune[knob] = value;
  return 0;
}

int aigv_tune_default(int knob, int value) {
  if (knob == AIGV_TUNE_CO_KMAX) return aigv_tune_co_gemm(value);
  if (!known(knob) || !KNOBS[knob].process_default)
    return fail(nullptr, AIGV_ERR_ARG, "aigv_tune_default: knob %d has no process default here (aigv_tune_gemm / _attention / _skinny set the others)", knob);
  if (!valid(knob, value)) return fail(nullptr, AIGV_ERR_ARG, "aigv_tune_default: value %d out of range for knob %d", value, knob);
  g_tune.v[knob] = value;
// ... 67 lines not shown
```

### aigv-assessor_amd/native.py

```python
from __future__ import annotations

import ctypes as C
import os
from typing import Optional

HERE = os.path.dirname(os.path.abspath(__file__))
LIB_PATH = os.environ.get("AIGV_AMD_LIB") or os.path.join(HERE, "libaigv_amd.so")
ABI_VERSION = 3


class NativeError(RuntimeError):
    pass


class AigvConfig(C.Structure):
    _fields_ = [
        ("vit_hidden", C.c_int32), ("vit_inter", C.c_int32), ("vit_heads", C.c_int32), ("vit_layers", C.c_int32),
        ("image_size", C.c_int32), ("patch_size", C.c_int32), ("num_channels", C.c_int32),
        ("vit_norm_rms", C.c_int32), ("vit_qk_norm", C.c_int32), ("vit_qkv_bias", C.c_int32),
        ("vit_eps", C.c_float), ("select_layer", C.c_int32), ("shuffle", C.c_int32),
        ("llm_hidden", C.c_int32), ("llm_inter", C.c_int32), ("llm_heads", C.c_int32), ("llm_kv_heads", C.c_int32),
        ("llm_layers", C.c_int32), ("vocab", C.c_int32), ("rms_eps", C.c_float), ("max_positions", C.c_int32),
        ("motion_dim", C.c_int32), ("n_score_layers", C.c_int32), ("score_dims", C.c_int32 * 8),
        ("max_frames", C.c_int32), ("vit_chunk", C.c_int32), ("max_tokens", C.c_int32), ("max_seqs", C.c_int32),
# ... 17 lines not shown
        check(n)
    ops = []
    for i in range(n):
        op = SlowFastOp()
        check(lib.aigv_slowfast_plan_op(handle, i, C.byref(op), C.sizeof(SlowFastOp)))
        ops.append(op)
    return ops


_P = C.c_void_p
_I = C.c_int
_F = C.c_float
_I64P = C.POINTER(C.c_int64)
_I32P = C.POINTER(C.c_int32)

PROTOTYPES = {
    "aigv_abi_version": (_I, []),
    "aigv_sizeof_config": (_I, []),
    "aigv_ctx_create": (_I, [_I, C.POINTER(AigvConfig), C.POINTER(_P)]),
    "aigv_ctx_destroy": (None, [_P]),
    "aigv_ctx_resize": (_I, [_P, C.POINTER(AigvConfig)]),
    "aigv_last_error": (C.c_char_p, [_P]),
    "aigv_clear_hip_error": (None, []),
    "aigv_load_weight": (_I, [_P, C.c_char_p, _P, _I64P, _I, _I, _I]),
    "aigv_finalize_weights": (_I, [_P]),
    "aigv_vit_forward": (_I, [_P, _P, _I, _P, _P]),
    "aigv_project": (_I, [_P, _P, _I, _P, _P]),
    "aigv_motion_project": (_I, [_P, _P, _I, _P, _P]),
    "aigv_llm_prefill": (_I, [_P, _P, _P, _I32P, _I, _P, _I, _P, _I32P, _P, _I32P, _I, _P, _I, _P]),
    "aigv_llm_extend": (_I, [_P, _P, _I32P, _I, _I32P, _P, _I32P, _I, _P, _I, _P]),
    "aigv_score_attention_arm": (_I, [_P, _I32P, _I, _P, _P, _I, _I, _P]),
    "aigv_score_attention_arm_tokens": (_I, [_P, _I32P, _I, _P, _P, _I, _I, _P, _P, _I]),
    "aigv_kv_fork": (_I, [_P, _I, _P]),
    "aigv_kv_reorder": (_I, [_P, _P, _P, _I, _P]),
    "aigv_set_row_trimming": (_I, [_P, _I]),
    "aigv_set_gemm_mode": (_I, [_P, _I]),
    "aigv_set_attention_numerics": (_I, [_P, _I]),
    "aigv_get_attention_numerics": (_I, [_P]),
    "aigv_ctx_tune": (_I, [_P, _I, _I]),
    "aigv_decode_step": (_I, [_P, _P, _P, _P]),
    "aigv_decode_step_logprob": (_I, [_P, _P, _P, _P, _P]),
    "aigv_decode_step_cand_logprob": (_I, [_P, _P, _P, _P, _P, _I, _P, _P]),
    "aigv_decode_step_topk_logprob": (_I, [_P, _P, _P, _P, _I, _P, _P, _P, _I, _P, _P]),
    "aigv_out_row_logits": (_I, [_P, _I, _I, _P, _I, _P]),
    "aigv_out_row_hidden": (_I, [_P, _I, _I, _P, _I, _P]),
    "aigv_out_row_logprob": (_I, [_P, _I, _I, _P, _P, _P]),
    "aigv_out_row_cand_logprob": (_I, [_P, _I, _I, _P, _I, _P, _P]),
    "aigv_out_row_topk_logprob": (_I, [_P, _I, _I, _I, _P, _P, _P]),
    "aigv_decode_eos": (_I, [_P, _P, _P, _I64P, _I, C.c_int64, _P]),
    "aigv_op_gemm": (_I, [_P, _I, _P, _I, _P, _I, _P, _P, _P, _I, _P, _I, _I, _I, _I, _I, _P]),
    "aigv_op_gemm_check": (_I, [_P, _I, _P, _I, _P, _I, _P, _P, _P, _I, _P, _I, _I, _I, _I, _I]),
    "aigv_op_skinny_gemm_check": (_I, [_P, _I, _I, _P, _I, _I, _I, _P, _I, _P, _I, _I]),
    "aigv_op_gemm_rows": (_I, [_P, _I, _P, _I, _P, _I, _P, _P, _P, _I, C.POINTER(C.c_int32), _I, _I, _I, _I, _P]),
    "aigv_op_gemm_splitk": (_I, [_P, _I, _P, _I, _P, _I, _P, _P, _P, _I, _I, _I, _I, _I, _I, _P, _P]),
    "aigv_op_gemm_splitk256": (_I, [_P, _I, _P, _I, _P, _I, _P, _P, _P, _I, _I, _I, _I, _I, _I, _P, _P]),
    "aigv_slowfast_create": (_I, [_I, _I, _I, _I, _I, C.POINTER(_P)]),
    "aigv_slowfast_destroy": (None, [_P]),
    "aigv_slowfast_load_weight": (_I, [_P, C.c_char_p, _P, C.POINTER(C.c_int64), _I, _I]),
    "aigv_slowfast_finalize": (_I, [_P]),
    "aigv_slowfast_forward": (_I, [_P, _P, _I, _P, _P]),
    "aigv_slowfast_flops_per_clip": (C.c_double, [_P]),
    "aigv_op_conv3d": (_I, [_P, _I, _I, _I, C.POINTER(_I), _P, _I, _P, _I, _P, _I, _P, _I, _I, _I, _P]),
    "aigv_slowfast_plan_size": (_I, [_P]),
    "aigv_slowfast_plan_op": (_I, [_P, _I, C.POINTER(SlowFastOp), _I]),
    "aigv_slowfast_run_ops": (_I, [_P, _P, _I, _P, _I, _I, _P]),
    "aigv_slowfast_buffer_read": (_I, [_P, _I, C.c_int64, _I, _P, _P]),
    "aigv_slowfast_buffer_write": (_I, [_P, _I, C.c_int64, _I, _P, _P]),
    "aigv_slowfast_slow_indices": (_I, [_I, _I32P]),
    "aigv_slowfast_pool_weights": (_I, [_I, _I, _I, _I, C.POINTER(_F), C.POINTER(_F), C.POINTER(_F)]),
    "aigv_slowfast_conv_k_slices": (_I, [C.c_int64, _I, _I]),
    "aigv_set_precision": (_I, [_P, _I]),
    "aigv_op_quant_fp8_rows": (_I, [_P, _I, _I, _I, _P, _I, _P, _P]),
    "aigv_op_gemm_fp8": (_I, [_P, _I, _P, _I, _P, _I, _P, _P, _P, _P, _P, _I, _I, _I, _I, _I, _I, _P, _P]),
    "aigv_op_skinny_gemm": (_I, [_P, _I, _I, _P, _I, _I, _I, _P, _P, _I, _P, _I, _I, _P]),
    "aigv_op_skinny_gemm_fp8": (_I, [_P, _I, _I, _P, _I, C.POINTER(C.c_float), _I, _I, _P, _I, _P, _I, _I, _P, _F, _I, _P]),
    "aigv_op_layernorm": (_I, [_P, _I, _P, _P, _P, _I, _I, _I, _F, _P]),
    "aigv_op_rmsnorm": (_I, [_P, _I, _P, _P, _I, _I, _I, _F, _P, _P]),
    "aigv_op_rope": (_I, [_P, _I, _P, _P, _P, _I, _I, _I, _I, _I, _P]),
    "aigv_op_attention": (_I, [_P, _I, _P, _I, _P, _I, _P, _I, _P, _I, _I, _I, _I, _I, _I, _I, _I, _F, _F, _P]),
    "aigv_op_attention_rope": (_I, [_P, _I, _P, _I, _P, _I, _P, _I, _P, _I, _I, _I, _I, _I, _I, _I, _I, _F, _F, _P, _P, _P, _P]),
    "aigv_op_attention_ex": (_I, [_P, _I, _P, _I, _P, _I, _P, _I, _P, _I, _I, _I, _I, _I, _I, C.c_int64, _P, _I, _I, _F, _F, _P, _P, _P, _I, _I, _P]),
    "aigv_op_attention_drop": (_I, [_P, _I, _P, _I, _P, _I, _P, _I, _P, _I, _I, _I, _I, _I, _I, C.c_int64, _P, _I, _I, _F, _F, _P, _P, _P, _I, _I, _P, _I, _P]),
    "aigv_key_drop_arm": (_I, [_P, _P, _I]),
    "aigv_key_drop_arm_ex": (_I, [_P, _P, _P, _I, _I, _I]),
    "aigv_depth_lens_arm": (_I, [_P, _I32P, _I, _I32P, _I, _P, _P, _P]),
    "aigv_depth_lens_token_readout": (_I, [_P, _P, _I, _I, _P, _I, _P, _P, _P, _P]),
    "aigv_stream_capture_arm": (_I, [_P, _I32P, _I, _I, _I, _P]),
    "aigv_stream_patch_arm": (_I, [_P, _I32P, _I, _I, _I, _P]),
    "aigv_head_capture_arm": (_I, [_P, _I32P, _I, _I, _I, _P]),
    "aigv_head_patch_arm": (_I, [_P, _I32P, _I, _I, _I, C.POINTER(C.c_uint64), _P]),
    "aigv_head_scale_arm": (_I, [_P, _I32P, _I, C.POINTER(C.c_float)]),
    "aigv_op_attention_drop_rows": (_I, [_P, _I, _P, _I, _P, _I, _P, _I, _P, _I, _I, _I, _I, _I, _I, C.c_int64, _P, _I, _I, _F, _F, _P, _P, _P, _I, _I, _P, _P, _I, _P]),
    "aigv_op_kv_store": (_I, [_P, _I, _P, _P, _P, _P, _I, _I, _I, _I, _I, _P]),
    "aigv_op_attention_probe": (_I, [_P, _I, _P, _I, _I32P, _I, _I, _I, _I, _I, C.c_int64, _I32P, _I, _P, _P, _I, _I32P, _I, _P, _P, _I, _I, _P, _P]),
    "aigv_op_attention_probe_tokens": (_I, [_P, _I, _P, _I, _I32P, _I, _I, _I, _I, _I, C.c_int64, _I32P, _I, _P, _P, _I, _I32P, _I, _P, _P, _I, _I, _P, _P, _I, _P]),
    "aigv_op_pixel_shuffle": (_I, [_P, _I, _I, _P, _I, _P]),
    "aigv_op_im2col": (_I, [_P, _I, _I, _I, _I, _I, _P, _P]),
    "aigv_op_lm_head_argmax": (_I, [_P, _I, _I, _P, _I, _P, _P, _P, _P]),
    "aigv_op_lm_head_argmax_logprob": (_I, [_P, _I, _I, _P, _I, _P, C.c_int64, _P, _P, _P, _P]),
    "aigv_op_lm_head_argmax_logprob_scratch_bytes": (C.c_int64, [_I, _I]),
    "aigv_op_label_logprob": (_I, [_P, _I, _I, _I, _P, _P, _P]),
    "aigv_op_cand_logprob": (_I, [_P, _I, _I, _I, _P, _I, _P, _P]),
    "aigv_op_lm_head_argmax_cand_logprob": (_I, [_P, _I, _I, _P, _I, _P, _I, _P, C.c_int64, _P, _P, _P, _P, _P]),
    "aigv_op_lm_head_argmax_cand_logprob_scratch_bytes": (C.c_int64, [_I, _I]),
    "aigv_op_topk_logprob": (_I, [_P, _I, _I, _I, _I, _P, _P, _P]),
    "aigv_op_lm_head_argmax_topk_logprob": (_I, [_P, _I, _I, _P, _I, _I, _P, _I, _P, C.c_int64, _P, _P, _P, _P, _P, _P, _P]),
# ... 128 lines not shown
```

### include/aigv_amd.h

```cpp
#ifndef AIGV_AMD_H
#define AIGV_AMD_H

#include <stdint.h>

#ifdef __cplusplus
extern "C" {
#endif

#define AIGV_ABI_VERSION 3

#define AIGV_MAX_CANDIDATES 64
#define AIGV_MAX_TOPK 16

#define AIGV_MAX_ATTN_SEGMENTS 64
#define AIGV_MAX_PROBE_ROWS 64

#define AIGV_MAX_KV_CAPACITY 262144

typedef struct aigv_ctx aigv_ctx;

enum aigv_status {
  AIGV_OK = 0,
  AIGV_ERR_ARG = -1,
  AIGV_ERR_HIP = -2,
// ... 176 lines not shown
int aigv_op_attention_decode_drop(const void* q, int ldq, int q_group_stride, const void* kc, const void* vc, const int32_t* kv_lens, int cap,
                                  void* o, int ldo, int n_seq, int n_kv, int g, int head_dim, float post_div, int max_kv_len, float* ws,
                                  int64_t ws_floats, const uint64_t* key_drop, int ld_drop, void* stream);
int aigv_op_skinny_rope_kv(const void* x, int ldx, int R, const void* W, int ldw, int N, int K, void* qkv, int ldo, const int32_t* pos,
                           const int32_t* seq, const void* cos, const void* sin, void* kc, void* vc, int g, int n_kv, int cap,
                           const void* norm_w, float eps, int p, void* stream);
int aigv_op_skinny_swiglu_normed(const void* x, int ldx, int R, const void* W, int ldw, int N, int K, void* out, int ldo,
                                 const void* norm_w, float eps, int p, void* stream);
int aigv_op_skinny_rope_kv_fp8(const void* x, int ldx, int R, const void* W_e4m3, int ldw, const float* w_scale, int N, int K, void* qkv,
                               int ldo, const int32_t* pos, const int32_t* seq, const void* cos, const void* sin, void* kc, void* vc, int g,
                               int n_kv, int cap, const void* norm_w, float eps, int p, void* stream);

int aigv_op_score_head(const void* x, int ldx, int B, int n_layers, const int32_t* dims_host, const void* const* w_dev, const void* const* b_dev,
                       void* scratch, int64_t scratch_bytes, float* score, void* stream);
int aigv_op_score_head_groups(const void* x, int ldx, int G, int64_t group_stride, int B, int n_layers, const int32_t* dims_host,
                              const void* const* w_dev, const void* const* b_dev, void* scratch, int64_t scratch_bytes, float* score, void* stream);
int aigv_op_lens_tap(const void* src, int ld, const int32_t* idx, int n, const void* w, void* raw, void* normed, int H, float eps, void* stream);
int aigv_op_rmsnorm_quant_fp8(const void* x, int ldx, const void* w, void* q_e4m3, int ldq, float* row_scale, int rows, int H, float eps, void* stream);
int aigv_op_rope_slots(void* qkv, int ld, const int32_t* pos, const void* cos, const void* sin, int tokens, int first_rot, int n_rot, int slots,
                       int n_groups, int head_dim, void* stream);
int aigv_op_embed(const int64_t* ids, const int32_t* slot, const void* emb, const void* vis, const void* motion, int n_vis, void* out, int tokens, int H,
                  void* stream);
int aigv_op_seqpos(const int32_t* cu_host, int n_seq, const int32_t* pos_offset_host, int32_t* pos, int32_t* seq, int32_t* cu_dev, int tokens, void* stream);
int aigv_op_gather_rows(const void* src, int ld, const int32_t* idx, int n, void* dst, int H, void* stream);
int aigv_op_scatter_rows(const void* src, const int32_t* idx, int n, void* dst, int ld, int H, void* stream);
int aigv_op_cls_rows(const void* cls_pos, void* x, int n_frames, int tokens_per_frame, int H, void* stream);
int aigv_op_write_ints(const int32_t* host, int n, int32_t* dst, void* stream);
int aigv_op_stream_rows(void* stream_rows, int ld, int T, const int32_t* rows_host, int n, int32_t* idx_dev, void* side, int n_depths, int depth, int H,
                        int to_stream, void* stream);
int aigv_op_head_rows(void* ao, int ld, int T, const int32_t* rows_host, int n, int32_t* idx_dev, void* side, int n_layers, int layer, int n_heads, int D,
                      int mode, uint64_t head_bits, const float* scale_host, void* stream);

int aigv_op_frame_ingest(const void* hwc_u8, int n_frames, int height, int width, const float* mean, const float* stdv,
                         void* out_nchw, void* stream);

int aigv_op_frame_resize_ingest(const void* hwc_u8, int n_frames, int in_h, int in_w, int out_h, int out_w, const float* mean,
                                const float* stdv, void* tmp_u8, void* out_u8_hwc, void* out_nchw, void* stream);

enum aigv_tune_knob {
  AIGV_TUNE_GEMM_MODE = 0,
  AIGV_TUNE_GEMM256_ORDER = 1,
  AIGV_TUNE_GEMM256_VARIANT = 2,
  AIGV_TUNE_ATTN_WAVES = 3,
  AIGV_TUNE_SKINNY_P = 4,
  AIGV_TUNE_BODY_TILE = 5,
  AIGV_TUNE_CO_KMAX = 6,
  AIGV_TUNE_TAIL_SLICES = 7,
  AIGV_TUNE_ATTN_LEAD_KEY = 8,
  AIGV_TUNE_DECODE_FUSED = 9,
  AIGV_TUNE_DECODE_FP8 = 10,
  AIGV_TUNE_SKINNY_P8 = 11,
  AIGV_TUNE_FUSE_TAILS = 12,
  AIGV_TUNE_LONE_BODY = 13,
  AIGV_TUNE_COUNT = 14
};
int aigv_ctx_tune(aigv_ctx* ctx, int knob, int value);
int aigv_tune_gemm(int mode, double rate256);
int aigv_tune_co_gemm(int kmax);
int aigv_tune_default(int knob, int value);
int aigv_plan_gemm(int M, int N, int K, int epi, int* plan, double* est_us);
enum {
  AIGV_ROUTE_128 = 1,
  AIGV_ROUTE_256 = 2,
  AIGV_ROUTE_CO = 4,
  AIGV_ROUTE_SPLITK_128 = 8,
  AIGV_ROUTE_SPLITK_256 = 16,
  AIGV_ROUTE_SKINNY = 32,
  AIGV_ROUTE_COLUMN_BAND = 64,
  AIGV_ROUTE_TAB_256 = 128,
  AIGV_ROUTE_TAB_SPLITK = 256,
  AIGV_ROUTE_TAB_FUSED = 512,
  AIGV_ROUTE_TAB_LONE = 1024,
  AIGV_ROUTE_TAB_128 = 2048,
  AIGV_ROUTE_TAB_CO = 4096,
  AIGV_ROUTE_TINY = 8192,
  AIGV_ROUTE_TINY_STRIDED = 16384
};
int aigv_gemm_route(int clear);
int aigv_tune_attention(int waves);
int aigv_tune_skinny(int p);

enum aigv_prof_class { AIGV_PROF_GEMM = 0, AIGV_PROF_ATTN_VIT = 1, AIGV_PROF_ATTN_LLM = 2, AIGV_PROF_SKINNY = 3,
                       AIGV_PROF_GEMM_FP8 = 4, AIGV_PROF_GEMM_VIT = 5, AIGV_PROF_COUNT = 6 };
int aigv_prof_enable(aigv_ctx* ctx, int on);
int aigv_prof_read(aigv_ctx* ctx, int cls, int64_t* launches, double* total_ms, double* flops, double* bytes);

typedef struct aigv_slowfast aigv_slowfast;
int aigv_slowfast_create(int device, int max_clips, int frames_per_clip, int height, int width, aigv_slowfast** out);
void aigv_slowfast_destroy(aigv_slowfast* sf);
int aigv_slowfast_load_weight(aigv_slowfast* sf, const char* name, const void* host_data, const int64_t* shape, int ndim, int dtype);
int aigv_slowfast_finalize(aigv_slowfast* sf);
int aigv_slowfast_forward(aigv_slowfast* sf, const void* frames_nchw_bf16, int clips, void* feature_bf16, void* stream);
double aigv_slowfast_flops_per_clip(const aigv_slowfast* sf);
int aigv_op_conv3d(const void* x, int ld_in, int Cin, int B, const int* dims, const void* w_packed, int Kp, const float* bias, int Cout,
                   const void* res, int ld_res, void* out, int ld_out, int c_off, int relu, void* stream);

#define AIGV_SF_BUFFERS 14
enum aigv_slowfast_op_kind { AIGV_SF_REPACK = 0, AIGV_SF_CONV = 1, AIGV_SF_MAXPOOL = 2, AIGV_SF_HEADPOOL = 3 };
typedef struct aigv_slowfast_op {
  int32_t kind;
  int32_t in_buf, res_buf, out_buf;
  int32_t out2_buf;
  int32_t pair_stem;
  int64_t in_elems, res_elems, out_elems, out2_elems;
  int32_t ld_in, Cin, Ti, Hi, Wi;
  int32_t kt, kh, kw, st, sh, sw, pt, ph, pw;
  int32_t To, Ho, Wo, Cout, Kp;
  int32_t ld_res, ld_out, c_off, relu;
  int32_t k_slices;
  int32_t T, H, W, C;
  int32_t window;
  int32_t reserved;
  char conv_name[128], norm_name[128];
} aigv_slowfast_op;
int aigv_slowfast_plan_size(const aigv_slowfast* sf);
int aigv_slowfast_plan_op(const aigv_slowfast* sf, int index, aigv_slowfast_op* op, int sizeof_op);
int aigv_slowfast_run_ops(aigv_slowfast* sf, const void* frames_nchw_bf16, int clips, void* feature_bf16, int first, int last, void* stream);
int aigv_slowfast_buffer_read(aigv_slowfast* sf, int buf, int64_t elems_per_clip, int clips, void* dst_bf16, void* stream);
int aigv_slowfast_buffer_write(aigv_slowfast* sf, int buf, int64_t elems_per_clip, int clips, const void* src_bf16, void* stream);
int aigv_slowfast_slow_indices(int frames_per_clip, int32_t* idx);
int aigv_slowfast_pool_weights(int frames, int H, int W, int window, float* wt, float* wy, float* wx);
int aigv_slowfast_conv_k_slices(int64_t rows, int CoutPad, int Kp);

#ifdef __cplusplus
}
#endif
#endif
```

Baseline: 35.30.

## Defer split-K tail finalize into the following RMSNorm or RoPE kernel

The split-K finalize for the ragged tail rows of the LLM row-plan GEMMs is now deferred instead of launched on its own. It is folded into the next consumer kernel: RMSNorm after the wo/w2 residual GEMMs, and RoPE after the QKV GEMM. New fused rmsnorm_fin and rope_fin kernels reduce the partial slabs for the tail rows before normalising or rotating, which removes one kernel launch and one round trip of the tail output through memory per fused GEMM. The cost is state tracking for the pending finalize, flush points around taps, fp8 and ViT paths, and a guard that split-K scratch is not reused while slabs are held. The behaviour is gated by a tune knob that defaults to on.

```diff
diff --git a/aigv-assessor_amd/context.py b/aigv-assessor_amd/context.py
--- a/aigv-assessor_amd/context.py
+++ b/aigv-assessor_amd/context.py
@@ -207,7 +207,8 @@
         self._ctx_set("aigv_set_gemm_mode", int(mode))
 
     TUNE_KNOBS = {"gemm_mode": 0, "gemm256_order": 1, "gemm256_variant": 2, "attn_waves": 3, "skinny_p": 4, "body_tile": 5, "co_kmax": 6,
-                  "tail_slices": 7, "attn_lead_key": 8, "decode_fused": 9, "decode_fp8": 10, "skinny_p8": 11, "fuse_tails": 12, "lone_body": 13}
+                  "tail_slices": 7, "attn_lead_key": 8, "decode_fused": 9, "decode_fp8": 10, "skinny_p8": 11, "fuse_tails": 12, "lone_body": 13,
+                  "fuse_finalize": 14}
 
     def tune(self, knob: str, value: int = -1):
         self._drop_graphs()
diff --git a/aigv-assessor_amd/csrc/ctx.h b/aigv-assessor_amd/csrc/ctx.h
--- a/aigv-assessor_amd/csrc/ctx.h
+++ b/aigv-assessor_amd/csrc/ctx.h
@@ -74,6 +74,7 @@
   uint8_t* q8 = nullptr;
   float* q8_scale = nullptr;
   aigv::RowPlan rp_vit, rp_llm;
+  PendingTail pend;
   const aigv::RowPlan* cur_rp = nullptr;
   bool trim_last_layer = true;
   int attn_round_scores = AIGV_ATTENTION_NUMERICS_DEFAULT;
@@ -252,12 +253,17 @@
                const bf16_t* resid, int ldr, bf16_t* out, int ldo, int epi, hipStream_t s, int p = 1);
 constexpr size_t SPLITK_MAX_FLOATS = (size_t)64 << 20;
 int splitk_scratch(aigv_ctx* c, size_t need_floats, float** out);
+PendingTail& pending_tail(aigv_ctx* c);
+void announce_tail_consumer(aigv_ctx* c, int consumer);
+const PendingTail* take_pending_tail(aigv_ctx* c, PendingTail* out);
+int flush_pending_finalize(aigv_ctx* c, hipStream_t s);
 
 struct DisarmScope {
   aigv_ctx* c;
   explicit DisarmScope(aigv_ctx* c_) : c(c_) {}
   ~DisarmScope() { c->probe.armed = false; c->drop.armed = false; c->lens.armed = false; c->stream_cap.armed = false; c->stream_patch.armed = false;
-                   c->head_cap.armed = false; c->head_patch.armed = false; c->head_scale.armed = false; }
+                   c->head_cap.armed = false; c->head_patch.armed = false; c->head_scale.armed = false;
+                   c->pend = PendingTail{}; }
 };
 int probe_plan(aigv_ctx* c, const char* op, const int32_t* cu, int B, const int32_t* off_host, ProbeArgs* out);
 int probe_layer(aigv_ctx* c, const ProbeArgs& plan, int li, bool cache, hipStream_t s);
diff --git a/aigv-assessor_amd/csrc/dispatch.hip b/aigv-assessor_amd/csrc/dispatch.hip
--- a/aigv-assessor_amd/csrc/dispatch.hip
+++ b/aigv-assessor_amd/csrc/dispatch.hip
@@ -35,7 +35,45 @@
 static float* g_op_splitk_ws[MAX_DEVICES] = {};
 static std::mutex g_op_splitk_lock;
 
+static PendingTail g_op_pend;
+
+PendingTail& pending_tail(aigv_ctx* c) { return c ? c->pend : g_op_pend; }
+
+void announce_tail_consumer(aigv_ctx* c, int consumer) { pending_tail(c).consumer = consumer; }
+
+const PendingTail* take_pending_tail(aigv_ctx* c, PendingTail* out) {
+  PendingTail& p = pending_tail(c);
+  p.consumer = TAIL_CONSUMER_NONE;
+  if (!p.pending) return nullptr;
+  *out = p;
+  p.pending = false;
+  took(AIGV_TAILFIN_CONSUMED);
+  return out;
+}
+
+int flush_pending_finalize(aigv_ctx* c, hipStream_t s) {
+  PendingTail& p = pending_tail(c);
+  p.consumer = TAIL_CONSUMER_NONE;
+  if (!p.pending) return 0;
+  p.pending = false;
+  HIPCHK(c, aigv_launch_gemm_finalize(p.f, p.epi, p.S, p.ws, s));
+  return 0;
+}
+
+static int finalize_or_defer(aigv_ctx* c, const GemmArgs& f, int epi, int S, const float* ws, hipStream_t s) {
+  PendingTail& p = pending_tail(c);
+  const bool fits = (p.consumer == TAIL_CONSUMER_ROPE && epi == EPI_STORE) || (p.consumer == TAIL_CONSUMER_RMSNORM && epi == EPI_RESID);
+  if (fits && tune_knob(c, AIGV_TUNE_FUSE_FINALIZE) == 0 && f.tab_halves <= TAIL_FIN_MAX_HALVES && !(c && (c->on_vit_front || c->fp8_llm))) {
+    p.pending = true; p.f = f; p.epi = epi; p.S = S; p.ws = ws;
+    took(AIGV_TAILFIN_DEFERRED);
+    return 0;
+  }
+  HIPCHK(c, aigv_launch_gemm_finalize(f, epi, S, ws, s));
+  return 0;
+}
+
 int splitk_scratch(aigv_ctx* c, size_t need_floats, float** out) {
+  if (pending_tail(c).pending && !(c && c->on_vit_front)) return fail(c, AIGV_ERR_STATE, "split-K scratch asked for while a deferred finalize still holds its slabs (flush_pending_finalize first)");
   if (need_floats > SPLITK_MAX_FLOATS) return fail(c, AIGV_ERR_ARG, "split-K scratch: %zu floats exceed the planner's cap", need_floats);
   if (c) {
     if (need_floats > c->splitk_floats) return fail(c, AIGV_ERR_STATE, "split-K scratch: %zu floats exceed the context's %zu", need_floats, c->splitk_floats);
@@ -279,7 +317,7 @@
   return best;
 }
 
-static int launch_tab(aigv_ctx* c, const GemmArgs& a, int epi, const int32_t* tab, int halves, int rows, int S, hipStream_t s) {
+static int launch_tab(aigv_ctx* c, const GemmArgs& a, int epi, const int32_t* tab, int halves, int rows, int S, hipStream_t s, bool may_defer = false) {
   if (halves <= 0) return 0;
   GemmArgs b = tuned(c, a);
   b.row_tab = tab; b.tab_halves = halves;
@@ -292,6 +330,12 @@
   float* ws = nullptr;
   TRY(splitk_scratch(c, (size_t)S * ((halves + 1) / 2) * 256 * a.N, &ws));
   took(AIGV_ROUTE_TAB_SPLITK);
+  if (may_defer && pending_tail(c).consumer != TAIL_CONSUMER_NONE && (a.K / 64) % S == 0 && epi != EPI_PATCH) {
+    GemmArgs p = b;
+    p.part = ws; p.k_slices = S;
+    HIPCHK(c, aigv_launch_gemm256_partial(p, s));
+    return finalize_or_defer(c, b, epi, S, ws, s);
+  }
   HIPCHK(c, aigv_launch_gemm_splitk(b, epi, S, ws, s, true));
   return 0;
 }
@@ -379,7 +423,7 @@
       HIPCHK(c, aigv_launch_gemm256_fused(b, epi, s));
       GemmArgs f = a;
       f.row_tab = rp.d_tab + 2 * rp.body_halves; f.tab_halves = rp.tail_halves;
-      HIPCHK(c, aigv_launch_gemm_finalize(f, epi, S, ws, s));
+      TRY(finalize_or_defer(c, f, epi, S, ws, s));
       return run_tiny_tails(c, a, epi, rp, s);
     }
     if (!lone) TRY(launch_tab(c, a, epi, rp.d_tab, rp.body_halves, rp.body_halves * 128, 1, s));
@@ -391,7 +435,7 @@
     if (max_halves < 2) return fail(c, AIGV_ERR_STATE, "split-K scratch too small for one tail tile (N=%d, %d slices)", a.N, S);
     for (int h0 = 0; h0 < rp.tail_halves; h0 += max_halves) {
       const int nh = std::min(max_halves, rp.tail_halves - h0);
-      TRY(launch_tab(c, a, epi, rp.d_tab + 2 * (rp.body_halves + h0), nh, nh * 128, S, s));
+      TRY(launch_tab(c, a, epi, rp.d_tab + 2 * (rp.body_halves + h0), nh, nh * 128, S, s, h0 == 0 && nh == rp.tail_halves));
     }
   }
   return run_tiny_tails(c, a, epi, rp, s);
@@ -480,6 +524,11 @@
   return 0;
 }
 
+extern "C" int aigv_plan_tail_slices(int N, int K) {
+  if (N <= 0 || K <= 0 || N % 128 || K % 64) return fail(nullptr, AIGV_ERR_ARG, "aigv_plan_tail_slices: bad problem N=%d K=%d", N, K);
+  return tail_slices(N, K, g_tune[AIGV_TUNE_TAIL_SLICES]);
+}
+
 extern "C" int aigv_gemm_route(int clear) {
   return (int)(clear ? g_route.exchange(0, std::memory_order_relaxed) : g_route.load(std::memory_order_relaxed));
 }
diff --git a/aigv-assessor_amd/csrc/kernels.h b/aigv-assessor_amd/csrc/kernels.h
--- a/aigv-assessor_amd/csrc/kernels.h
+++ b/aigv-assessor_amd/csrc/kernels.h
@@ -48,6 +48,15 @@
 bool aigv_gemm256_supported(const GemmArgs& a);
 hipError_t aigv_launch_gemm256_fused(const GemmArgs& a, int epi, hipStream_t s);
 hipError_t aigv_launch_gemm_finalize(const GemmArgs& a, int epi, int k_slices, const float* ws, hipStream_t s);
+enum { TAIL_CONSUMER_NONE = 0, TAIL_CONSUMER_ROPE = 1, TAIL_CONSUMER_RMSNORM = 2 };
+constexpr int TAIL_FIN_MAX_HALVES = 32;
+struct PendingTail {
+  int consumer = TAIL_CONSUMER_NONE;
+  bool pending = false;
+  GemmArgs f{};
+  int epi = 0, S = 0;
+  const float* ws = nullptr;
+};
 hipError_t aigv_launch_gemm256(const GemmArgs& a, int epi, hipStream_t s);
 bool aigv_gemmco_supported(const GemmArgs& a);
 hipError_t aigv_launch_gemmco(const GemmArgs& a, int epi, hipStream_t s);
@@ -125,7 +134,7 @@
 hipError_t aigv_launch_layernorm(const bf16_t* x, int ldx, const bf16_t* w, const bf16_t* b, bf16_t* y, int ldy,
                                  int rows, int H, float eps, hipStream_t s);
 hipError_t aigv_launch_rmsnorm(const bf16_t* x, int ldx, const bf16_t* w, bf16_t* y, int ldy, int rows, int H,
-                               float eps, const int32_t* row_idx, hipStream_t s);
+                               float eps, const int32_t* row_idx, hipStream_t s, const PendingTail* tail = nullptr);
 hipError_t aigv_launch_pixel_shuffle(const bf16_t* vit, int grid, int Hv, bf16_t* out, int frames, hipStream_t s);
 hipError_t aigv_launch_im2col(const bf16_t* frames, int F, int C, int S, int P, int Kp, bf16_t* out, hipStream_t s);
 hipError_t aigv_launch_gather_rows(const bf16_t* src, int ld, const int32_t* idx, int n, bf16_t* dst, int H, hipStream_t s);
@@ -141,7 +150,7 @@
                                  uint64_t heads, const float* scale, hipStream_t s);
 hipError_t aigv_launch_cls_rows(const bf16_t* cls_pos, bf16_t* x, int F, int tokens_per_frame, int H, hipStream_t s);
 hipError_t aigv_launch_rope(bf16_t* qkv, int ld, const int32_t* pos, const bf16_t* cos, const bf16_t* sin,
-                            int tokens, int n_rot, int slots, int n_groups, int D, hipStream_t s, int first_rot = 0);
+                            int tokens, int n_rot, int slots, int n_groups, int D, hipStream_t s, int first_rot = 0, const PendingTail* tail = nullptr);
 hipError_t aigv_launch_embed(const int64_t* ids, const int32_t* slot, const bf16_t* emb, const bf16_t* vis,
                              const bf16_t* motion, int n_vis, bf16_t* out, int tokens, int H, hipStream_t s);
 enum { SK_STORE = 0, SK_RESID = 1, SK_SWIGLU = 2, SK_GELU = 3, SK_ARGMAX = 4, SK_RELU = 5, SK_LS_RESID = 6, SK_ROPE_KV = 7, SK_ARGMAX_LSE = 8, SK_ARGMAX_LSE_STORE = 9 };
diff --git a/aigv-assessor_amd/csrc/ops.hip b/aigv-assessor_amd/csrc/ops.hip
--- a/aigv-assessor_amd/csrc/ops.hip
+++ b/aigv-assessor_amd/csrc/ops.hip
@@ -1,3 +1,4 @@
+#include <functional>
 #include "ctx.h"
 
 using namespace aigv;
@@ -45,6 +46,59 @@
   hipStreamSynchronize((hipStream_t)stream);
   hipFree(rp.d_tab);
   return rc;
+}
+
+static int op_gemm_rows_then(const char* op, const GemmArgs& a, int epi, const int32_t* cu_host, int n_seq, int consumer_kind, hipStream_t s,
+                             const std::function<hipError_t(const PendingTail*)>& consumer) {
+  if (!cu_host || n_seq < 1 || cu_host[0] != 0) return fail(nullptr, AIGV_ERR_ARG, "%s: bad cu_seqlens", op);
+  for (int b = 0; b < n_seq; ++b)
+    if (cu_host[b + 1] <= cu_host[b]) return fail(nullptr, AIGV_ERR_ARG, "%s: empty sequence %d", op, b);
+  if (a.M != cu_host[n_seq]) return fail(nullptr, AIGV_ERR_ARG, "%s: the sequences hold %d rows, the operands %d", op, cu_host[n_seq], a.M);
+  RowPlan rp;
+  rp.cap_halves = a.M / 128 + 2 * n_seq + 2;
+  HIPCHK(nullptr, hipMalloc((void**)&rp.d_tab, (size_t)2 * rp.cap_halves * sizeof(int32_t)));
+  int rc = build_row_plan(nullptr, rp, cu_host, n_seq, s);
+  if (!rc) {
+    announce_tail_consumer(nullptr, consumer_kind);
+    rc = run_gemm_rows(nullptr, a, epi, rp, s);
+  }
+  PendingTail pt;
+  const PendingTail* tail = take_pending_tail(nullptr, &pt);
+  if (!rc) {
+    const hipError_t e = consumer(tail);
+    if (e != hipSuccess) rc = fail(nullptr, e == hipErrorInvalidValue ? AIGV_ERR_ARG : AIGV_ERR_HIP, "%s: the row pass: %s", op, hipGetErrorString(e));
+  }
+  hipStreamSynchronize(s);
+  hipFree(rp.d_tab);
+  return rc;
+}
+
+int aigv_op_gemm_rows_rmsnorm(const void* A, int lda, const void* W_, int ldw, void* C, int ldc, const void* bias, const void* resid, int ldr,
+                              const int32_t* cu_host, int n_seq, int N, int K, const void* norm_w, void* y, int ldy, float eps, void* stream) {
+  const char* op = "aigv_op_gemm_rows_rmsnorm";
+  if (!cu_host || n_seq < 1 || !norm_w || !y) return fail(nullptr, AIGV_ERR_ARG, "%s: null argument", op);
+  const int M = cu_host[n_seq];
+  GemmArgs a = gemm_args((const bf16_t*)A, lda, (const bf16_t*)W_, ldw, (bf16_t*)C, ldc, M, N, K);
+  a.bias = (const bf16_t*)bias; a.resid = (const bf16_t*)resid; a.ldr = ldr;
+  if (ldy < N || ldy % 8 || N % 8 || N > 16384) return fail(nullptr, AIGV_ERR_ARG, "%s: the norm needs N = %d a multiple of 8 up to 16384 and ldy = %d a multiple of 8, >= N", op, N, ldy);
+  return op_gemm_rows_then(op, a, EPI_RESID, cu_host, n_seq, TAIL_CONSUMER_RMSNORM, (hipStream_t)stream, [&](const PendingTail* tail) {
+    return aigv_launch_rmsnorm((const bf16_t*)C, ldc, (const bf16_t*)norm_w, (bf16_t*)y, ldy, M, N, eps, nullptr, (hipStream_t)stream, tail);
+  });
+}
+
+int aigv_op_gemm_rows_rope(const void* A, int lda, const void* W_, int ldw, void* C, int ldc, const void* bias, const int32_t* cu_host, int n_seq, int N, int K,
+                           const int32_t* pos, const void* cos, const void* sin, int first_rot, int n_rot, int slots, int n_groups, int head_dim, void* stream) {
+  const char* op = "aigv_op_gemm_rows_rope";
+  if (!cu_host || n_seq < 1 || !pos || !cos || !sin) return fail(nullptr, AIGV_ERR_ARG, "%s: null argument", op);
+  if (head_dim < 16 || head_dim % 16 || n_groups < 1 || slots < 1 || first_rot < 0 || n_rot < 1 || (int64_t)first_rot + n_rot > slots ||
+      (int64_t)n_groups * slots * head_dim > N)
+    return fail(nullptr, AIGV_ERR_ARG, "%s: needs head_dim a multiple of 16, 0 <= first_rot, first_rot + n_rot <= slots and n_groups slots head_dim <= N", op);
+  const int M = cu_host[n_seq];
+  GemmArgs a = gemm_args((const bf16_t*)A, lda, (const bf16_t*)W_, ldw, (bf16_t*)C, ldc, M, N, K);
+  a.bias = (const bf16_t*)bias;
+  return op_gemm_rows_then(op, a, EPI_STORE, cu_host, n_seq, TAIL_CONSUMER_ROPE, (hipStream_t)stream, [&](const PendingTail* tail) {
+    return aigv_launch_rope((bf16_t*)C, ldc, pos, (const bf16_t*)cos, (const bf16_t*)sin, M, n_rot, slots, n_groups, head_dim, (hipStream_t)stream, first_rot, tail);
+  });
 }
 
 int aigv_op_gemm_splitk(const void* A, int lda, const void* W_, int ldw, void* C, int ldc, const void* bias, const void* ls,
diff --git a/aigv-assessor_amd/csrc/passes.hip b/aigv-assessor_amd/csrc/passes.hip
--- a/aigv-assessor_amd/csrc/passes.hip
+++ b/aigv-assessor_amd/csrc/passes.hip
@@ -192,18 +192,21 @@
   const aigv_config& k = c->cfg;
   const LlmLayer& L = c->llm[li];
   const int H = k.llm_hidden, D = c->head_dim, g = c->g, nkv = k.llm_kv_heads;
+  PendingTail pt;
   if (c->fp8_llm) {
+    TRY(flush_pending_finalize(c, s));
     HIPCHK(c, aigv_launch_rmsnorm_quant_fp8(c->l_h, H, L.an, c->q8, H, c->q8_scale, T, H, k.rms_eps, s));
     TRY(run_gemm_fp8(c, nullptr, H, H, c->llm8[li].wqkv, c->llm8[li].s_wqkv, c->l_qkv, c->qkv_out, T, c->qkv_out, EPI_STORE, nullptr, 0, s));
   } else {
-    HIPCHK(c, aigv_launch_rmsnorm(c->l_h, H, L.an, c->l_t, H, T, H, k.rms_eps, nullptr, s));
+    HIPCHK(c, aigv_launch_rmsnorm(c->l_h, H, L.an, c->l_t, H, T, H, k.rms_eps, nullptr, s, take_pending_tail(c, &pt)));
+    announce_tail_consumer(c, TAIL_CONSUMER_ROPE);
     TRY(run_llm_gemm(c, gemm_args(c->l_t, H, L.wqkv, H, c->l_qkv, c->qkv_out, T, c->qkv_out, H), EPI_STORE, s));
   }
-  HIPCHK(c, aigv_launch_rope(c->l_qkv, c->qkv_out, c->l_pos, c->rope_cos, c->rope_sin, T, 1, g + 2, nkv, D, s, g));
-  return 0;
-}
-
-static int llm_layer_post(aigv_ctx* c, int li, int T, hipStream_t s) {
+  HIPCHK(c, aigv_launch_rope(c->l_qkv, c->qkv_out, c->l_pos, c->rope_cos, c->rope_sin, T, 1, g + 2, nkv, D, s, g, take_pending_tail(c, &pt)));
+  return 0;
+}
+
+static int llm_layer_post(aigv_ctx* c, int li, int T, hipStream_t s, bool defer_w2 = false) {
   const aigv_config& k = c->cfg;
   const LlmLayer& L = c->llm[li];
   const int H = k.llm_hidden, I = k.llm_inter;
@@ -218,13 +221,17 @@
   {
     GemmArgs a = gemm_args(c->l_ao, H, L.wo, H, c->l_h, H, T, H, H);
     a.resid = c->l_h; a.ldr = H;
+    announce_tail_consumer(c, TAIL_CONSUMER_RMSNORM);
     TRY(run_llm_gemm(c, a, EPI_RESID, s));
   }
-  HIPCHK(c, aigv_launch_rmsnorm(c->l_h, H, L.fn, c->l_t, H, T, H, k.rms_eps, nullptr, s));
+  PendingTail pt;
+  HIPCHK(c, aigv_launch_rmsnorm(c->l_h, H, L.fn, c->l_t, H, T, H, k.rms_eps, nullptr, s, take_pending_tail(c, &pt)));
   TRY(run_llm_gemm(c, gemm_args(c->l_t, H, L.w13, H, c->l_ffn, I, T, 2 * I, H), EPI_SWIGLU, s));
   GemmArgs a = gemm_args(c->l_ffn, I, L.w2, I, c->l_h, H, T, H, I);
   a.resid = c->l_h; a.ldr = H;
+  if (defer_w2) announce_tail_consumer(c, TAIL_CONSUMER_RMSNORM);
   TRY(run_llm_gemm(c, a, EPI_RESID, s));
+  if (!defer_w2) TRY(flush_pending_finalize(c, s));
   return 0;
 }
 
@@ -384,8 +391,10 @@
   double attn_flops = 0;
   for (int b = 0; b < B; ++b) { const double L = cu[b + 1] - cu[b]; attn_flops += 4.0 * (L * (L + 1) / 2) * D * k.llm_heads; }
   const size_t kv_layer = (size_t)k.max_seqs * nkv * k.kv_capacity * D;
+  const bool taps_l_h = patching || capturing || lensing;
   for (int li = 0; li < k.llm_layers; ++li) {
     const LlmLayer& L = c->llm[li];
+    if (taps_l_h) TRY(flush_pending_finalize(c, s));
     if (patching && li >= sp.lo && li < sp.hi)
       HIPCHK(c, aigv_launch_stream_rows(c->l_h, H, c->l_streamidx, (int)sp.rows.size(), sp.buf, sp.hi - sp.lo, li - sp.lo, H, true, s));
     if (capturing && li >= sc.lo && li < sc.hi)
@@ -442,9 +451,10 @@
       if (lensing) TRY(lens_tap(k.llm_layers, c->l_h, lens_idx));
       break;
     }
-    TRY(llm_layer_post(c, li, T, s));
+    TRY(llm_layer_post(c, li, T, s, !taps_l_h && li + 1 < k.llm_layers));
     if (lensing && li == k.llm_layers - 1) TRY(lens_tap(k.llm_layers, c->l_h, lens_idx));
   }
+  TRY(flush_pending_finalize(c, s));
   if (!trim) TRY(final_rows(c, score, B, R, argmax, c->l_h, false, s));
   if (lensing && c->lens.n_score > 0) {
     const int nS = c->lens.n_score, per = std::max(1, 64 / nS);
@@ -613,6 +623,7 @@
   HIPCHK(c, aigv_launch_write_ints(c->h_kvlen.data(), B, c->l_kvlen, s));
   HIPCHK(c, aigv_launch_embed(ids, c->l_neg1, c->tok_emb, nullptr, nullptr, 0, c->l_h, T, H, s));
   TRY(upload_out_rows(c, score_rows, score != nullptr, B, logit_rows, R, T, s));
+  TRY(flush_pending_finalize(c, s));
   ProbeArgs probe{};
   if (probing) TRY(probe_plan(c, "aigv_llm_extend", cu, B, c->h_kvlen.data(), &probe));
   double attn_flops = 0;
diff --git a/aigv-assessor_amd/csrc/rowops.hip b/aigv-assessor_amd/csrc/rowops.hip
--- a/aigv-assessor_amd/csrc/rowops.hip
+++ b/aigv-assessor_amd/csrc/rowops.hip
@@ -1,5 +1,6 @@
 #include <algorithm>
 #include "common.h"
+#include "epilogue.h"
 #include "kernels.h"
 
 namespace {
@@ -124,6 +125,56 @@
   AIGV_RMSNORM_ROW(src, ld, srow, w, normed, H, row, H, eps, AIGV_LENS_KEEP_RAW)
 #undef AIGV_LENS_KEEP_RAW
 }
+template <int EPI, int SC>
+__device__ __forceinline__ u16x4 tail_fin4(const GemmArgs& p, const float* __restrict__ part, int S, size_t slab, int sm, int m, int n) {
+  static_assert(EPI == EPI_STORE || EPI == EPI_RESID, "the consumers finish STORE (RoPE) and RESID (RMSNorm) tails");
+  f32x4 a = *(const f32x4*)(part + (size_t)sm * p.N + n);
+  if constexpr (SC > 0) {
+    f32x4 b[SC - 1];
+#pragma unroll
+    for (int sidx = 1; sidx < SC; ++sidx) b[sidx - 1] = *(const f32x4*)(part + sidx * slab + (size_t)sm * p.N + n);
+#pragma unroll
+    for (int sidx = 1; sidx < SC; ++sidx)
+#pragma unroll
+      for (int e = 0; e < 4; ++e) a[e] += b[sidx - 1][e];
+  } else {
+    for (int sidx = 1; sidx < S; ++sidx) {
+      const f32x4 b = *(const f32x4*)(part + sidx * slab + (size_t)sm * p.N + n);
+#pragma unroll
+      for (int e = 0; e < 4; ++e) a[e] += b[e];
+    }
+  }
+  const u16x4 zero = {0, 0, 0, 0};
+  const u16x4 v = epi_acc4<EPI>(a, p.bias != nullptr, p.bias ? *(const u16x4*)(p.bias + n) : zero, zero);
+  if constexpr (EPI == EPI_RESID) return epi_row4<EPI>(v, *(const u16x4*)(p.resid + (size_t)m * p.ldr + n));
+  else return v;
+}
+
+template <int SC>
+__global__ __launch_bounds__(256) void rmsnorm_fin_kernel(const GemmArgs p, const float* __restrict__ part, int S,
+                                                          const bf16_t* __restrict__ w, bf16_t* __restrict__ y, int ldy, int H, float eps) {
+  int n_tail = 0;
+  for (int h = 0; h < p.tab_halves; ++h) n_tail += p.row_tab[2 * h + 1];
+  int row = (int)blockIdx.x - n_tail, sm = -1;
+  if (row < 0) {
+    int r = blockIdx.x;
+    for (int h = 0; h < p.tab_halves; ++h) {
+      const int cnt = p.row_tab[2 * h + 1];
+      if (sm < 0 && r < cnt) { sm = h * 128 + r; row = p.row_tab[2 * h] + r; }
+      r -= cnt;
+    }
+  } else {
+    for (int h = 0; h < p.tab_halves; ++h)
+      if (row >= p.row_tab[2 * h]) row += p.row_tab[2 * h + 1];
+  }
+  if (sm >= 0) {
+    const size_t slab = (size_t)((p.tab_halves + 1) / 2) * 256 * p.N;
+    for (int n = threadIdx.x * 4; n < p.N; n += 1024) *(u16x4*)(p.C + (size_t)row * p.ldc + n) = tail_fin4<EPI_RESID, SC>(p, part, S, slab, sm, row, n);
+    __syncthreads();
+  }
+  const bf16_t* x = p.C;
+  AIGV_RMSNORM_ROW(x, p.ldc, row, w, y, ldy, row, H, eps, AIGV_RMSNORM_NO_RAW)
+}
 #undef AIGV_RMSNORM_ROW
 #undef AIGV_RMSNORM_NO_RAW
 
@@ -290,6 +341,56 @@
   }
 }
 
+template <int SC>
+__global__ __launch_bounds__(256) void rope_fin_kernel(const GemmArgs p, const float* __restrict__ part, int S, int body_blocks,
+                                                       const int32_t* __restrict__ pos, const bf16_t* __restrict__ cs, const bf16_t* __restrict__ sn,
+                                                       int tokens, int n_rot, int slots, int n_groups, int D, int first_rot) {
+  __shared__ int tab[2 * TAIL_FIN_MAX_HALVES];
+  const int half = D >> 1, cph = half >> 3;
+  const int per_tok = n_groups * n_rot * cph;
+  bf16_t* qkv = p.C;
+  const int ld = p.ldc;
+  auto rotate = [&](int t, int r) {
+    const int c = r % cph; r /= cph;
+    const int s = r % n_rot, gidx = r / n_rot;
+    bf16_t* base = qkv + (size_t)t * ld + (size_t)(gidx * slots + first_rot + s) * D + (c << 3);
+    const size_t tb = (size_t)pos[t] * half + (c << 3);
+    const u16x8 lo = *(const u16x8*)base, hi = *(const u16x8*)(base + half);
+    const u16x8 co = *(const u16x8*)(cs + tb), si = *(const u16x8*)(sn + tb);
+    u16x8 olo, ohi;
+#pragma unroll
+    for (int e = 0; e < 8; ++e) {
+      bf16_t a, b;
+      rope_pair(lo[e], hi[e], co[e], si[e], a, b);
+      olo[e] = a;
+      ohi[e] = b;
+    }
+    *(u16x8*)base = olo;
+    *(u16x8*)(base + half) = ohi;
+  };
+  const int tail_blocks = p.tab_halves * 128;
+  if ((int)blockIdx.x >= tail_blocks) {
+    if ((int)threadIdx.x < 2 * p.tab_halves) tab[threadIdx.x] = p.row_tab[threadIdx.x];
+    __syncthreads();
+    const size_t total = (size_t)tokens * per_tok;
+    for (size_t i = (size_t)(blockIdx.x - tail_blocks) * 256 + threadIdx.x; i < total; i += (size_t)body_blocks * 256) {
+      const int t = (int)(i / per_tok);
+      bool in_tail = false;
+      for (int h = 0; h < p.tab_halves; ++h) in_tail |= (unsigned)(t - tab[2 * h]) < (unsigned)tab[2 * h + 1];
+      if (!in_tail) rotate(t, (int)(i - (size_t)t * per_tok));
+    }
+    return;
+  }
+  const int sm = (int)blockIdx.x, h = sm >> 7, r = sm & 127;
+  if (r >= p.row_tab[2 * h + 1]) return;
+  const int m = p.row_tab[2 * h] + r;
+  const size_t slab = (size_t)((p.tab_halves + 1) / 2) * 256 * p.N;
+  for (int n = threadIdx.x * 4; n < p.N; n += 1024) *(u16x4*)(qkv + (size_t)m * ld + n) = tail_fin4<EPI_STORE, SC>(p, part, S, slab, sm, m, n);
+  __syncthreads();
+  if (m < tokens)
+    for (int i = threadIdx.x; i < per_tok; i += 256) rotate(m, i);
+}
+
 __global__ __launch_bounds__(256) void embed_kernel(const int64_t* __restrict__ ids, const int32_t* __restrict__ slot,
                                                     const bf16_t* __restrict__ emb, const bf16_t* __restrict__ vis,
                                                     const bf16_t* __restrict__ motion, int n_vis,
@@ -489,7 +590,19 @@
 }
 
 hipError_t aigv_launch_rmsnorm(const bf16_t* x, int ldx, const bf16_t* w, bf16_t* y, int ldy, int rows, int H,
-                               float eps, const int32_t* row_idx, hipStream_t s) {
+                               float eps, const int32_t* row_idx, hipStream_t s, const PendingTail* tail) {
+  if (tail) {
+    const GemmArgs& f = tail->f;
+    if (!tail->pending || tail->epi != EPI_RESID || tail->S < 2 || !tail->ws || !f.row_tab || f.tab_halves < 1 || f.tab_halves > TAIL_FIN_MAX_HALVES ||
+        f.C != x || f.ldc != ldx || f.N != H || f.M != rows || row_idx || !f.resid || f.N % 4 || f.ldc % 4 || f.ldr % 4 || rows <= 0 || H % 8 || H > MAXC * 256 * 8)
+      return hipErrorInvalidValue;
+    auto go = [&](auto kernel) { hipLaunchKernelGGL(kernel, dim3(rows), dim3(256), 0, s, f, tail->ws, tail->S, w, y, ldy, H, eps); };
+    if (tail->S == 2) go(rmsnorm_fin_kernel<2>);
+    else if (tail->S == 4) go(rmsnorm_fin_kernel<4>);
+    else if (tail->S == 8) go(rmsnorm_fin_kernel<8>);
+    else go(rmsnorm_fin_kernel<0>);
+    return hipGetLastError();
+  }
   if (rows <= 0) return hipSuccess;
   if (H % 8 || H > MAXC * 256 * 8) return hipErrorInvalidValue;
   hipLaunchKernelGGL(rmsnorm_kernel, dim3(rows), dim3(256), 0, s, x, ldx, w, y, ldy, H, eps, row_idx);
@@ -582,7 +695,25 @@
 }
 
 hipError_t aigv_launch_rope(bf16_t* qkv, int ld, const int32_t* pos, const bf16_t* cos, const bf16_t* sin,
-                            int tokens, int n_rot, int slots, int n_groups, int D, hipStream_t s, int first_rot) {
+                            int tokens, int n_rot, int slots, int n_groups, int D, hipStream_t s, int first_rot, const PendingTail* tail) {
+  if (tail) {
+    const GemmArgs& f = tail->f;
+    if (!tail->pending || tail->epi != EPI_STORE || tail->S < 2 || !tail->ws || !f.row_tab || f.tab_halves < 1 || f.tab_halves > TAIL_FIN_MAX_HALVES ||
+        f.C != qkv || f.ldc != ld || f.M != tokens || f.N % 4 || f.ldc % 4 || tokens <= 0 || n_rot <= 0 || D % 16 || first_rot < 0 || first_rot + n_rot > slots ||
+        (long)n_groups * slots * D > f.N)
+      return hipErrorInvalidValue;
+    const size_t total = (size_t)tokens * n_groups * n_rot * (D / 16);
+    const int body_blocks = (int)((total + 255) / 256 < 4096 ? (total + 255) / 256 : 4096);
+    auto go = [&](auto kernel) {
+      hipLaunchKernelGGL(kernel, dim3(body_blocks + f.tab_halves * 128), dim3(256), 0, s, f, tail->ws, tail->S, body_blocks, pos, cos, sin, tokens, n_rot, slots,
+                         n_groups, D, first_rot);
+    };
+    if (tail->S == 2) go(rope_fin_kernel<2>);
+    else if (tail->S == 4) go(rope_fin_kernel<4>);
+    else if (tail->S == 8) go(rope_fin_kernel<8>);
+    else go(rope_fin_kernel<0>);
+    return hipGetLastError();
+  }
   if (tokens <= 0 || n_rot <= 0) return hipSuccess;
   if (D % 16 || first_rot < 0 || first_rot + n_rot > slots) return hipErrorInvalidValue;
   const size_t total = (size_t)tokens * n_groups * n_rot * (D / 16);
diff --git a/aigv-assessor_amd/csrc/tune.hip b/aigv-assessor_amd/csrc/tune.hip
--- a/aigv-assessor_amd/csrc/tune.hip
+++ b/aigv-assessor_amd/csrc/tune.hip
@@ -30,8 +30,9 @@
     {0, 0, in_forms, false},
     {0, 2, nullptr, true},
     {1, 4, nullptr, true},
+    {0, 1, nullptr, true},
 };
-static_assert(AIGV_TUNE_GEMM_MODE == 0 && AIGV_TUNE_CO_KMAX == 6 && AIGV_TUNE_LONE_BODY == 13 && AIGV_TUNE_COUNT == 14, "KNOBS follows the enum's order");
+static_assert(AIGV_TUNE_GEMM_MODE == 0 && AIGV_TUNE_CO_KMAX == 6 && AIGV_TUNE_LONE_BODY == 13 && AIGV_TUNE_FUSE_FINALIZE == 14 && AIGV_TUNE_COUNT == 15, "KNOBS follows the enum's order");
 
 constexpr Tune library_defaults() {
   Tune t{};
diff --git a/aigv-assessor_amd/native.py b/aigv-assessor_amd/native.py
--- a/aigv-assessor_amd/native.py
+++ b/aigv-assessor_amd/native.py
@@ -93,6 +93,9 @@
     "aigv_op_gemm_check": (_I, [_P, _I, _P, _I, _P, _I, _P, _P, _P, _I, _P, _I, _I, _I, _I, _I]),
     "aigv_op_skinny_gemm_check": (_I, [_P, _I, _I, _P, _I, _I, _I, _P, _I, _P, _I, _I]),
     "aigv_op_gemm_rows": (_I, [_P, _I, _P, _I, _P, _I, _P, _P, _P, _I, C.POINTER(C.c_int32), _I, _I, _I, _I, _P]),
+    "aigv_op_gemm_rows_rmsnorm": (_I, [_P, _I, _P, _I, _P, _I, _P, _P, _I, C.POINTER(C.c_int32), _I, _I, _I, _P, _P, _I, C.c_float, _P]),
+    "aigv_op_gemm_rows_rope": (_I, [_P, _I, _P, _I, _P, _I, _P, C.POINTER(C.c_int32), _I, _I, _I, _P, _P, _P, _I, _I, _I, _I, _I, _P]),
+    "aigv_plan_tail_slices": (_I, [_I, _I]),
     "aigv_op_gemm_splitk": (_I, [_P, _I, _P, _I, _P, _I, _P, _P, _P, _I, _I, _I, _I, _I, _I, _P, _P]),
     "aigv_op_gemm_splitk256": (_I, [_P, _I, _P, _I, _P, _I, _P, _P, _P, _I, _I, _I, _I, _I, _I, _P, _P]),
     "aigv_slowfast_create": (_I, [_I, _I, _I, _I, _I, C.POINTER(_P)]),
diff --git a/include/aigv_amd.h b/include/aigv_amd.h
--- a/include/aigv_amd.h
+++ b/include/aigv_amd.h
@@ -252,7 +252,8 @@
   AIGV_TUNE_SKINNY_P8 = 11,
   AIGV_TUNE_FUSE_TAILS = 12,
   AIGV_TUNE_LONE_BODY = 13,
-  AIGV_TUNE_COUNT = 14
+  AIGV_TUNE_FUSE_FINALIZE = 14,
+  AIGV_TUNE_COUNT = 15
 };
 int aigv_ctx_tune(aigv_ctx* ctx, int knob, int value);
 int aigv_tune_gemm(int mode, double rate256);
@@ -276,7 +277,16 @@
   AIGV_ROUTE_TINY = 8192,
   AIGV_ROUTE_TINY_STRIDED = 16384
 };
+enum aigv_gemm_tail_finalize {
+  AIGV_TAILFIN_DEFERRED = 32768,
+  AIGV_TAILFIN_CONSUMED = 65536
+};
 int aigv_gemm_route(int clear);
+int aigv_plan_tail_slices(int N, int K);
+int aigv_op_gemm_rows_rmsnorm(const void* A, int lda, const void* W, int ldw, void* C, int ldc, const void* bias, const void* resid, int ldr,
+                              const int32_t* cu_host, int n_seq, int N, int K, const void* norm_w, void* y, int ldy, float eps, void* stream);
+int aigv_op_gemm_rows_rope(const void* A, int lda, const void* W, int ldw, void* C, int ldc, const void* bias, const int32_t* cu_host, int n_seq, int N, int K,
+                           const int32_t* pos, const void* cos, const void* sin, int first_rot, int n_rot, int slots, int n_groups, int head_dim, void* stream);
 int aigv_tune_attention(int waves);
 int aigv_tune_skinny(int p);
 
```

Result: no change. 35.28 (-0.0%).
